# halide/Halide

Measured on AMD Instinct MI355X. Metric: megapixels/sec local_laplacian 8-level fp32 4K, higher is better.
Workload: dtype f32; 1 GPU; apps/local_laplacian J=8 levels=8 alpha=1/7 beta=1, u16 RGB planar 3840x2160; distinct_frames_per_gpu=8, lut_cached=True, streams_per_gpu=4, frame_scheduling=4 frame-queue streams, boundary=C ABI local_laplacian(halide_buffer_t*,int32,float,float,halide_buffer_t*), rccl_ranks=1, parallelism=frames sharded over 1 GPU(s), no data-path collective

## Files before the change

### halide_amd/csrc/local_laplacian.hip

```cpp
#include "hlmi_device_math.h"
#include "hlmi_internal.h"

#include <atomic>
#include <mutex>
#include <optional>
#include <stdlib.h>
#include <string.h>
#include <type_traits>

using namespace hlmi;

namespace {

constexpr int J = 8;
constexpr int MAX_K = 32;
constexpr int STRIP = 126;
constexpr int KCH = 8;
constexpr int D0_THREADS = 256;

struct Level {
    int lox, loy;
    int w, h;
    int ws;
    size_t ps;
    int rx0, rx1, ry0, ry1;
    bool odd;
    int nsx;
};

#ifndef HLMI_LL_PROBE
#define HLMI_LL_PROBE 0
#endif
#if HLMI_LL_PROBE
__device__ unsigned long long g_probe[32];
#define LL_PROBE_T(var) const unsigned long long var = wall_clock64()
#define LL_PROBE_ADD(slot, val) do { if ((threadIdx.x & 63) == 0) atomicAdd(&g_probe[slot], (unsigned long long)(val)); } while (0)
#else
#define LL_PROBE_T(var)
#define LL_PROBE_ADD(slot, val)
#endif

#ifndef HLMI_LL_RESIDENCY
#define HLMI_LL_RESIDENCY 0
#endif
#if HLMI_LL_RESIDENCY
__device__ int g_res[2][4096];
__device__ unsigned long long g_res_hist[16];
struct ResidencyProbe {
    int kind, slot;
    bool on;
    __device__ explicit ResidencyProbe(int k) : kind(k), slot(0), on(threadIdx.x == 0) {
        if (on) {
            unsigned hw, xcc;
            asm volatile("s_getreg_b32 %0, hwreg(HW_REG_HW_ID)" : "=s"(hw));
            asm volatile("s_getreg_b32 %0, hwreg(HW_REG_XCC_ID)" : "=s"(xcc));
            slot = (int)(((xcc & 0xfu) << 8) | ((hw >> 8) & 0xffu));
            const int own = atomicAdd(&g_res[kind][slot], 1);
            const int other = atomicAdd(&g_res[1 - kind][slot], 0);
            atomicAdd(&g_res_hist[8 * kind + min(other, 3)], 1ull);
            atomicAdd(&g_res_hist[8 * kind + 4 + min(own, 3)], 1ull);
        }
    }
    __device__ ~ResidencyProbe() {
        if (on) atomicSub(&g_res[kind][slot], 1);
    }
};
#define LL_RESIDENCY(kind) ResidencyProbe residency_probe_(kind)
#else
#define LL_RESIDENCY(kind)
#endif

struct Geometry {
    int K, half;
    float Km1, inv_Km1;
    int ix0, ix1, iy0, iy1;
};

__global__ void ll_remap_lut(float *lut, int half, float alpha) {
    int i = blockIdx.x * blockDim.x + threadIdx.x;
    if (i > 2 * half) return;
    float fx = (float)(i - half) * (1.0f / 256.0f);
    lut[i] = (alpha * fx) * dev::halide_exp(((-fx) * fx) * 0.5f);
}

__device__ __forceinline__ int xcd_block() {
    const int nb8 = gridDim.x >> 3, b = blockIdx.x;
    return (b < (nb8 << 3)) ? (b & 7) * nb8 + (b >> 3) : b;
}

__device__ __forceinline__ float down4(float a, float b, float c, float d) {
    return (dev::mad(3.0f, b + c, a) + d) * 0.125f;
}
__device__ __forceinline__ float down4_raw(float a, float b, float c, float d) { return dev::mad(3.0f, b + c, a) + d; }
__device__ __forceinline__ float down4_tail(float a, float b, float c, float d) {
    return (dev::mad(3.0f, b + c, a) + d) * 0.015625f;
}

__device__ __forceinline__ float gray_from(uint16_t r, uint16_t g, uint16_t b) {
    constexpr float s = (float)(1.0 / 65535.0);
    constexpr float C0 = (float)((double)s * (double)0.299f), C1 = (float)((double)s * (double)0.587f),
                    C2 = (float)((double)s * (double)0.114f);
    return dev::mad((float)b, C2, dev::mad2((float)r, C0, (float)g, C1));
}
__device__ __forceinline__ int idx_of(float gray, float Km1, int half) {
    return dev::clampi((int)((gray * Km1) * 256.0f), 0, half);
}
template<bool B1 = false>
__device__ __forceinline__ float g0_val(float gray, float level, float beta, float l) {
    return B1 ? ((gray - level) + level) + l : dev::mad(beta, gray - level, level) + l;
}

__device__ __forceinline__ float lane_prev(float v) {
    return __builtin_bit_cast(float, __builtin_amdgcn_update_dpp(0, __builtin_bit_cast(int, v), 0x138, 0xf, 0xf, true));
}
__device__ __forceinline__ float lane_next(float v) {
    return __builtin_bit_cast(float, __builtin_amdgcn_update_dpp(0, __builtin_bit_cast(int, v), 0x130, 0xf, 0xf, true));
}
__global__ void ll_dpp_probe(int *ok) {
    float v = (float)threadIdx.x;
    float p = lane_prev(v), n = lane_next(v);
    bool good = (threadIdx.x == 0 || p == v - 1.0f) && (threadIdx.x == 63 || n == v + 1.0f);
    unsigned long long m = __ballot(good);
    if (threadIdx.x == 0) *ok = (m == ~0ull) ? 1 : 0;
}

template<bool ODD>
__device__ __forceinline__ float2 hpair(const float (&dy)[4]) {
    if (!ODD) {
        float left = lane_prev(dy[3]);
        float right = lane_next(dy[0]);
        float o0 = down4_tail(left, dy[0], dy[1], dy[2]);
        float o1 = down4_tail(dy[1], dy[2], dy[3], right);
        float o2 = lane_next(o0);
        return make_float2(o1, o2);
    } else {
        float r0 = lane_next(dy[0]), r1 = lane_next(dy[1]);
        float o0 = down4_tail(dy[0], dy[1], dy[2], dy[3]);
        float o1 = down4_tail(dy[2], dy[3], r0, r1);
        return make_float2(o0, o1);
    }
}

struct QuadSel {
    int oq;
    int sel[4];
    bool plain;
};
__device__ __forceinline__ QuadSel quad_sel(int o, int w) {
    QuadSel q;
    q.oq = dev::clampi(o, 0, (w - 1) & ~3);
#pragma unroll
    for (int i = 0; i < 4; i++) q.sel[i] = dev::clampi(o + i, 0, w - 1) - q.oq;
    q.plain = (o >= 0) && (o + 3 <= w - 1);
    return q;
}
template<typename T>
__device__ __forceinline__ T pick4(T x, T y, T z, T w, int s) {
    T lo = (s & 1) ? y : x, hi = (s & 1) ? w : z;
    return (s & 2) ? hi : lo;
}

typedef unsigned short us4_t __attribute__((ext_vector_type(4)));
template<bool NT = false>
__device__ __forceinline__ ushort4 ld_frame4(const uint16_t *p) {
    if (NT) {
        us4_t v = __builtin_nontemporal_load(reinterpret_cast<const us4_t *>(p));
        return make_ushort4(v.x, v.y, v.z, v.w);
    }
    return *reinterpret_cast<const ushort4 *>(p);
}
template<bool NT = false>
__device__ __forceinline__ ushort2 ld_frame2(const void *sbase, uint32_t byte_off) {
    const uint32_t *q = reinterpret_cast<const uint32_t *>(reinterpret_cast<const char *>(sbase) + byte_off);
    const uint32_t w = NT ? __builtin_nontemporal_load(q) : *q;
    return make_ushort2((uint16_t)(w & 0xffffu), (uint16_t)(w >> 16));
}
template<bool NT = false>
__device__ __forceinline__ void st_frame2(void *p, uint16_t a, uint16_t b) {
    const uint32_t w = (uint32_t)a | ((uint32_t)b << 16);
    if (NT) __builtin_nontemporal_store(w, reinterpret_cast<uint32_t *>(p));
    else *reinterpret_cast<uint32_t *>(p) = w;
}

struct Raw {
    ushort4 c0, c1, c2;
};
struct Levels {
    float v[MAX_K];
};

template<bool VEC, bool NT = false>
__device__ __forceinline__ void load_raw(Raw &r, const uint16_t *__restrict__ rp, long co0, long co1, long co2,
                                         int oq, const int (&xo)[4]) {
    if (VEC) {
        r.c0 = ld_frame4<NT>(rp + co0 + oq);
        r.c1 = ld_frame4<NT>(rp + co1 + oq);
        r.c2 = ld_frame4<NT>(rp + co2 + oq);
    } else {
        r.c0 = make_ushort4(rp[co0 + xo[0]], rp[co0 + xo[1]], rp[co0 + xo[2]], rp[co0 + xo[3]]);
        r.c1 = make_ushort4(rp[co1 + xo[0]], rp[co1 + xo[1]], rp[co1 + xo[2]], rp[co1 + xo[3]]);
        r.c2 = make_ushort4(rp[co2 + xo[0]], rp[co2 + xo[1]], rp[co2 + xo[2]], rp[co2 + xo[3]]);
    }
}

template<bool ODD, bool VEC, bool LUT_LDS, bool B1>
__global__ __launch_bounds__(D0_THREADS, 2) void ll_down0(const uint16_t *__restrict__ in, long in_sy, long co0, long co1,
                                                   long co2, Geometry gm, Levels lev, float beta,
                                                   const float *__restrict__ lut_g, float *__restrict__ g1, int Xs,
                                                   int loy1, int w1, int h1, int ws1, size_t ps1, int nsx, int nsy,
                                                   int nunits) {
    extern __shared__ float slut[];
    if (LUT_LDS) {
        for (int i = threadIdx.x; i <= 2 * gm.half; i += D0_THREADS) slut[i] = lut_g[i];
        __syncthreads();
    }
    const float *lut = LUT_LDS ? slut : lut_g;
    const int wave = __builtin_amdgcn_readfirstlane(threadIdx.x >> 6);
    const int unit = xcd_block() * (D0_THREADS / 64) + wave;
    if (unit >= nunits) return;
    const int lane = threadIdx.x & 63;
    const int sy = unit % nsy, sx = unit / nsy;
    const int off = STRIP * sx + 2 * lane;
    const int P = Xs + off;
    const int q0 = ODD ? 2 * P - 1 : 2 * P - 2;
    const int iw = gm.ix1 - gm.ix0 + 1, ih = gm.iy1 - gm.iy0;
    const QuadSel qs = quad_sel(q0 - gm.ix0, iw);
    int xo[4];
#pragma unroll
    for (int i = 0; i < 4; i++) xo[i] = qs.oq + qs.sel[i];
    const bool edge_wave = VEC && __any(!qs.plain);
    const bool store_ok = (lane < 63) && (off < w1);
    const int t0 = (int)((long)sy * h1 / nsy), t1 = (int)((long)(sy + 1) * h1 / nsy) - 1;

    auto row_ptr = [&](int y_abs) -> const uint16_t * {
        return in + (long)(dev::clampi(y_abs - gm.iy0, 0, ih)) * in_sy;
    };

    for (int kb = 0; kb < gm.K; kb += KCH) {
        const int nk = min(KCH, gm.K - kb);
        const bool with_in = (kb == 0);
        const int lbase = gm.half - 256 * (kb + KCH - 1);
        float level[KCH];
#pragma unroll
        for (int kk = 0; kk < KCH; kk++) {
            const float lk = (float)(kb + kk) * gm.inv_Km1;
            level[kk] = kb + kk < MAX_K ? lev.v[kb + kk]
                                        : __builtin_bit_cast(float, __builtin_amdgcn_readfirstlane(__builtin_bit_cast(int, lk)));
            asm volatile("" : "+s"(level[kk]));
        }

        float a[KCH + 1][4], b[KCH + 1][4], a2[KCH + 1][4], b2[KCH + 1][4];
        auto gray_row = [&](const Raw &r, float (&gr)[4], int (&li)[4]) {
            const uint16_t rr[4] = {r.c0.x, r.c0.y, r.c0.z, r.c0.w};
            const uint16_t gg[4] = {r.c1.x, r.c1.y, r.c1.z, r.c1.w};
            const uint16_t bb[4] = {r.c2.x, r.c2.y, r.c2.z, r.c2.w};
            float g[4];
#pragma unroll
            for (int i = 0; i < 4; i++) g[i] = gray_from(rr[i], gg[i], bb[i]);
            if (edge_wave) {
#pragma unroll
                for (int i = 0; i < 4; i++) gr[i] = pick4(g[0], g[1], g[2], g[3], qs.sel[i]);
            } else {
#pragma unroll
                for (int i = 0; i < 4; i++) gr[i] = g[i];
            }
#pragma unroll
            for (int i = 0; i < 4; i++) li[i] = idx_of(gr[i], gm.Km1, gm.half) + lbase;
        };
        auto lut_issue = [&](int kk, const int (&l0)[4], const int (&l1)[4], float (&dst)[8]) {
#pragma unroll
            for (int i = 0; i < 4; i++) {
                dst[i] = lut[l0[i] + 256 * (KCH - 1 - kk)];
                dst[4 + i] = lut[l1[i] + 256 * (KCH - 1 - kk)];
            }
        };
        auto for_planes = [&](const float (&g0r)[4], const int (&l0)[4], const float (&g1r)[4], const int (&l1)[4],
                              auto &&F, auto &&G) {
            float lv[2][8];
            lut_issue(0, l0, l1, lv[0]);
#pragma unroll
            for (int kk = 0; kk <= KCH; kk++) {
                if (kk + 1 < KCH && kk + 1 < nk) lut_issue(kk + 1, l0, l1, lv[(kk + 1) & 1]);
                __builtin_amdgcn_sched_barrier(0);
                if (kk < KCH ? (kk < nk) : with_in) {
#pragma unroll
                    for (int i = 0; i < 4; i++) {
                        float v0 = kk < KCH ? g0_val<B1>(g0r[i], level[kk < KCH ? kk : 0], beta, lv[kk & 1][i]) : g0r[i];
                        float v1 = kk < KCH ? g0_val<B1>(g1r[i], level[kk < KCH ? kk : 0], beta, lv[kk & 1][4 + i]) : g1r[i];
                        F(kk, i, v0, v1);
                    }
                    G(kk);
                }
                __builtin_amdgcn_sched_barrier(0);
            }
        };

        const int T0 = loy1 + t0;
        {
            Raw ra, rb;
            load_raw<VEC>(ra, row_ptr(2 * T0 - 1), co0, co1, co2, qs.oq, xo);
            load_raw<VEC>(rb, row_ptr(2 * T0), co0, co1, co2, qs.oq, xo);
            float gra[4], grb[4];
            int la[4], lb[4];
            gray_row(ra, gra, la);
            gray_row(rb, grb, lb);
            for_planes(gra, la, grb, lb, [&](int kk, int i, float v0, float v1) { a[kk][i] = v0, b[kk][i] = v1; },
                       [&](int) {});
        }
        struct RowPair {
            float g0[4], g1[4];
        };
        Raw rc, rd;
        auto lut_pos = [&](const float (&g)[4], int (&l)[4]) {
#pragma unroll
            for (int i = 0; i < 4; i++) l[i] = idx_of(g[i], gm.Km1, gm.half) + lbase;
        };
        float2 *stage = reinterpret_cast<float2 *>(slut + (LUT_LDS ? ((2 * gm.half + 1 + 1) & ~1) : 0)) + threadIdx.x;
        auto step = [&](int t, const RowPair &cur, RowPair &nxt, float (&ia)[KCH + 1][4], float (&ib)[KCH + 1][4],
                        float (&oa)[KCH + 1][4], float (&ob)[KCH + 1][4]) {
            const int T = loy1 + t;
            int l0[4], l1[4];
            lut_pos(cur.g0, l0);
            lut_pos(cur.g1, l1);
            float dy[4];
            for_planes(cur.g0, l0, cur.g1, l1,
                       [&](int kk, int i, float cv, float dv) {
                           dy[i] = down4_raw(ia[kk][i], ib[kk][i], cv, dv);
                           oa[kk][i] = cv;
                           ob[kk][i] = dv;
                       },
                       [&](int kk) { stage[kk * D0_THREADS] = hpair<ODD>(dy); });
            if (t < t1) {
                int unused[4];
                gray_row(rc, nxt.g0, unused);
                gray_row(rd, nxt.g1, unused);
            }
            __builtin_amdgcn_sched_barrier(0);
            float *drow = g1 + (size_t)t * ws1 + off;
#pragma unroll
            for (int kk = 0; kk <= KCH; kk++) {
                if (kk < KCH ? (kk < nk) : with_in) {
                    const int plane = (kk < KCH) ? kb + kk : gm.K;
                    const float2 o = stage[kk * D0_THREADS];
                    if (store_ok) {
                        *reinterpret_cast<float2 *>(drow + (size_t)plane * ps1) = o;
                    }
                }
            }
            __builtin_amdgcn_sched_barrier(0);
            if (t + 1 < t1) {
                load_raw<VEC>(rc, row_ptr(2 * T + 5), co0, co1, co2, qs.oq, xo);
                load_raw<VEC>(rd, row_ptr(2 * T + 6), co0, co1, co2, qs.oq, xo);
            }
            __builtin_amdgcn_sched_barrier(0);
        };
        RowPair p0, p1;
        load_raw<VEC>(rc, row_ptr(2 * T0 + 1), co0, co1, co2, qs.oq, xo);
        load_raw<VEC>(rd, row_ptr(2 * T0 + 2), co0, co1, co2, qs.oq, xo);
        {
            int unused[4];
            gray_row(rc, p0.g0, unused);
            gray_row(rd, p0.g1, unused);
        }
        if (t0 < t1) {
            load_raw<VEC>(rc, row_ptr(2 * T0 + 3), co0, co1, co2, qs.oq, xo);
            load_raw<VEC>(rd, row_ptr(2 * T0 + 4), co0, co1, co2, qs.oq, xo);
        }
        for (int t = t0; t <= t1;) {
            step(t, p0, p1, a, b, a2, b2);
            if (++t > t1) break;
            step(t, p1, p0, a2, b2, a, b);
            ++t;
        }
    }
}

struct D01Args {
    const uint16_t *in;
    long in_sy, co0, co1, co2;
    float beta;
    const float *lut_g;
    float *g1;
    int so1, loy1, w1, h1, ws1;
    size_t ps1;
    float *g2;
    int so2, loy2, w2, h2, ws2;
    size_t ps2;
    int Pbase, S2, nsx, nsy, nunits;
    unsigned nsy_magic;
    int rows_base, rows_rem;
};
constexpr int D01_STATE = 2 * (KCH + 1) * 64;

template<bool ODD0, bool ODD1, bool B1, bool EXCH>
__global__ __launch_bounds__(D0_THREADS, 2) void ll_down01f(D01Args p, Geometry gm, Levels lev) {
    extern __shared__ float slut[];
    LL_PROBE_T(pt0);
    for (int i = threadIdx.x; i <= 2 * gm.half; i += D0_THREADS) slut[i] = p.lut_g[i];
    __syncthreads();
    LL_PROBE_T(pt1);
    const int wave = __builtin_amdgcn_readfirstlane(threadIdx.x >> 6);
    const int lane = threadIdx.x & 63;
    int sx, A, B;
    bool self_halo = true;
    bool publish = false;
    if (EXCH) {
        const int wg = xcd_block();
        sx = p.nsy_magic ? (int)__umulhi((unsigned)wg, p.nsy_magic) : wg;
        const int gy = wg - sx * p.nsy;
        const int GA = p.loy2 + gy * p.rows_base + min(gy, p.rows_rem);
        const int GB = GA + p.rows_base + (gy < p.rows_rem ? 1 : 0) - 1;
        const int n = (GB - GA + 1 + 1 + 3) >> 2;
        A = GA + wave * n, B = min(A + n - 1, GB);
        if (A > GB) {
            __syncthreads();
            return;
        }
        self_halo = !(wave < 3 && A + n <= GB);
        publish = wave > 0;
    } else {
        const int unit = xcd_block() * (D0_THREADS / 64) + wave;
        if (unit >= p.nunits) return;
        sx = p.nsy_magic ? (int)__umulhi((unsigned)unit, p.nsy_magic) : unit;
        const int sy = unit - sx * p.nsy;
        A = p.loy2 + sy * p.rows_base + min(sy, p.rows_rem);
        B = A + p.rows_base + (sy < p.rows_rem ? 1 : 0) - 1;
    }
    const int P = p.Pbase + 2 * p.S2 * sx + 2 * lane;
    const int q0 = ODD0 ? 2 * P - 1 : 2 * P - 2;
    const int iw = gm.ix1 - gm.ix0 + 1, ih = gm.iy1 - gm.iy0;
    const QuadSel qs = quad_sel(q0 - gm.ix0, iw);
    int xo[4];
#pragma unroll
    for (int i = 0; i < 4; i++) xo[i] = qs.oq + qs.sel[i];
    const bool edge_wave = __any(!qs.plain);
    const int T0 = 2 * A - 1, T1 = self_halo ? 2 * B + 2 : 2 * B;
    const int Ts0 = max(EXCH ? 2 * A - 1 : 2 * A, p.loy1), Ts1 = min(EXCH ? 2 * B : 2 * B + 1, p.loy1 + p.h1 - 1);
    const int off1 = P - p.so1;
    const bool st1_ok = lane < p.S2 && off1 >= 0 && off1 < p.w1;
    const int X2 = ODD1 ? (P + 1) >> 1 : P >> 1;
    const int off2 = X2 - p.so2;
    const bool st2_ok = (ODD1 ? lane < p.S2 : (lane >= 1 && lane <= p.S2)) && off2 >= 0 && off2 < p.w2;
    float2 *st2 = reinterpret_cast<float2 *>(slut + ((2 * gm.half + 2) & ~1)) + wave * D01_STATE + lane;
    float2 *pub_all = reinterpret_cast<float2 *>(slut + ((2 * gm.half + 2) & ~1)) + (D0_THREADS / 64) * D01_STATE + lane;
    float2 *pub_mine = pub_all + (wave - 1) * D01_STATE, *pub_next = pub_all + wave * D01_STATE;
    const int lbase = gm.half - 256 * (KCH - 1);
    float level[KCH];
#pragma unroll
    for (int kk = 0; kk < KCH; kk++) {
        level[kk] = lev.v[kk];
        asm volatile("" : "+v"(level[kk]));
    }
    auto walk = [&](auto edge_tag) {
    constexpr bool EDGE = decltype(edge_tag)::value;
#if HLMI_LL_PROBE
    unsigned long long pr_a0 = 0, pr_a = 0, pr_3 = 0;
#endif
    auto load_row = [&](Raw &r, int y_abs) {
        const uint16_t *rp = p.in + (long)(dev::clampi(y_abs - gm.iy0, 0, ih)) * p.in_sy;
        load_raw<true>(r, rp, p.co0, p.co1, p.co2, qs.oq, xo);
    };
    auto u16s = [&](const ushort4 &c, uint16_t (&o)[4]) {
        const uint2 w = __builtin_bit_cast(uint2, c);
        o[0] = (uint16_t)(w.x & 0xffffu), o[1] = (uint16_t)(w.x >> 16);
        o[2] = (uint16_t)(w.y & 0xffffu), o[3] = (uint16_t)(w.y >> 16);
    };
    struct Row {
        float g[4];
        int l[4];
    };
    auto prep_row = [&](const Raw &r, Row &o) {
        uint16_t rr[4], gg[4], bb[4];
        u16s(r.c0, rr), u16s(r.c1, gg), u16s(r.c2, bb);
#pragma unroll
        for (int i = 0; i < 4; i++) o.g[i] = gray_from(rr[i], gg[i], bb[i]);
        if (EDGE) {
            const float g0 = o.g[0], g1v = o.g[1], g2v = o.g[2], g3 = o.g[3];
#pragma unroll
            for (int i = 0; i < 4; i++) o.g[i] = pick4(g0, g1v, g2v, g3, qs.sel[i]);
        }
#pragma unroll
        for (int i = 0; i < 4; i++) {
            o.l[i] = (min((int)((o.g[i] * gm.Km1) * 256.0f), gm.half) + lbase) * 4;
            asm volatile("" : "+v"(o.l[i]));
        }
    };
    auto lut_issue = [&](int kk, const Row &r0, const Row &r1, float (&dst)[8]) {
#pragma unroll
        for (int i = 0; i < 4; i++) {
            dst[i] = *reinterpret_cast<const float *>(reinterpret_cast<const char *>(slut) + r0.l[i] + 1024 * (KCH - 1 - kk));
            dst[4 + i] = *reinterpret_cast<const float *>(reinterpret_cast<const char *>(slut) + r1.l[i] + 1024 * (KCH - 1 - kk));
        }
    };
    auto plane_vals = [&](int kk, const Row &r0, const Row &r1, const float (&lv)[8], float (&v0)[4], float (&v1)[4]) {
        if (kk < KCH) {
            const float L = level[kk < KCH ? kk : 0];
            float t[8];
#pragma unroll
            for (int i = 0; i < 4; i++) t[i] = r0.g[i] - L, t[4 + i] = r1.g[i] - L;
            if (!B1 && !dev::CANON_FMA) {
#pragma unroll
                for (int i = 0; i < 8; i++) t[i] = p.beta * t[i];
            }
#pragma unroll
            for (int i = 0; i < 8; i++) t[i] = (!B1 && dev::CANON_FMA) ? __builtin_fmaf(p.beta, t[i], L) : t[i] + L;
#pragma unroll
            for (int i = 0; i < 4; i++) v0[i] = t[i] + lv[i], v1[i] = t[4 + i] + lv[4 + i];
        } else {
#pragma unroll
            for (int i = 0; i < 4; i++) v0[i] = r0.g[i], v1[i] = r1.g[i];
        }
    };
    auto vpass = [&](const float (&ia)[4], const float (&ib)[4], const float (&c)[4], const float (&d)[4], float (&o)[4]) {
        float t[4];
#pragma unroll
        for (int i = 0; i < 4; i++) t[i] = ib[i] + c[i];
        if (!dev::CANON_FMA) {
#pragma unroll
            for (int i = 0; i < 4; i++) t[i] = 3.0f * t[i];
        }
#pragma unroll
        for (int i = 0; i < 4; i++) t[i] = dev::CANON_FMA ? __builtin_fmaf(3.0f, t[i], ia[i]) : ia[i] + t[i];
#pragma unroll
        for (int i = 0; i < 4; i++) o[i] = t[i] + d[i];
    };

    float a[KCH + 1][4], b[KCH + 1][4], a2[KCH + 1][4], b2[KCH + 1][4];
    Raw rc, rd;
    {
        Raw ra, rb;
        load_row(ra, 2 * T0 - 1);
        load_row(rb, 2 * T0);
        load_row(rc, 2 * T0 + 1);
        load_row(rd, 2 * T0 + 2);
#if HLMI_LL_PROBE
        LL_PROBE_T(ptA0);
        asm volatile("s_waitcnt vmcnt(0)" ::: "memory");
        LL_PROBE_T(ptA);
        pr_a0 = ptA0, pr_a = ptA;
#endif
        Row r0, r1;
        prep_row(ra, r0);
        prep_row(rb, r1);
        float lv[2][8];
        lut_issue(0, r0, r1, lv[0]);
#pragma unroll
        for (int kk = 0; kk <= KCH; kk++) {
            if (kk + 1 < KCH) lut_issue(kk + 1, r0, r1, lv[(kk + 1) & 1]);
            __builtin_amdgcn_sched_barrier(0);
            plane_vals(kk, r0, r1, lv[kk & 1], a[kk], b[kk]);
            __builtin_amdgcn_sched_barrier(0);
        }
    }
    auto step = [&](auto ph_tag, int T, const Row &c0, const Row &c1, Row &n0, Row &n1, float (&ia)[KCH + 1][4],
                    float (&ib)[KCH + 1][4], float (&oa)[KCH + 1][4], float (&ob)[KCH + 1][4], float2 *pub) {
        constexpr int PH = decltype(ph_tag)::value;
        float lv[2][8], dy[2][4];
        float2 res[KCH + 1];
        float2 sa, sb;
        const bool out2 = PH == 1 && T >= 2 * A + 2;
        float *d2 = p.g2 + (size_t)(((T - 2) >> 1) - p.loy2) * p.ws2 + off2;
        auto level2 = [&](int k) {
            const float2 c = res[k];
            if (PH == 0) {
                float2 pc;
                pc.x = dev::mad(3.0f, sb.x + c.x, sa.x);
                pc.y = dev::mad(3.0f, sb.y + c.y, sa.y);
                st2[(2 * k + 1) * 64] = pc;
                st2[(2 * k) * 64] = c;
            } else {
                const float rx = sb.x + c.x, ry = sb.y + c.y;
                float o;
                if (ODD1) {
                    const float nx = lane_next(rx), ny = lane_next(ry);
                    o = down4_tail(rx, ry, nx, ny);
                } else {
                    const float py = lane_prev(ry), nx = lane_next(rx);
                    o = down4_tail(py, rx, ry, nx);
                }
                if (out2 && st2_ok) d2[(size_t)k * p.ps2] = o;
                st2[(2 * k + 1) * 64] = c;
            }
        };
        auto state_issue = [&](int k) {
            if (PH == 0) sa = st2[(2 * k) * 64];
            sb = st2[(2 * k + 1) * 64];
        };
        lut_issue(0, c0, c1, lv[0]);
#pragma unroll
        for (int kk = 0; kk <= KCH; kk++) {
            if (kk > 0) state_issue(kk - 1);
            __builtin_amdgcn_sched_barrier(0);
            if (kk + 1 < KCH) lut_issue(kk + 1, c0, c1, lv[(kk + 1) & 1]);
            __builtin_amdgcn_sched_barrier(0);
            plane_vals(kk, c0, c1, lv[kk & 1], oa[kk], ob[kk]);
            vpass(ia[kk], ib[kk], oa[kk], ob[kk], dy[kk & 1]);
            if (kk > 0) {
                res[kk - 1] = hpair<ODD0>(dy[(kk - 1) & 1]);
                level2(kk - 1);
            }
            __builtin_amdgcn_sched_barrier(0);
        }
        state_issue(KCH);
        res[KCH] = hpair<ODD0>(dy[KCH & 1]);
        level2(KCH);
        prep_row(rc, n0);
        prep_row(rd, n1);
        __builtin_amdgcn_sched_barrier(0);
        if (T >= Ts0 && T <= Ts1) {
            float *drow = p.g1 + (size_t)(T - p.loy1) * p.ws1 + off1;
            if (st1_ok) {
#pragma unroll
                for (int kk = 0; kk <= KCH; kk++) *reinterpret_cast<float2 *>(drow + (size_t)kk * p.ps1) = res[kk];
            }
        }
        if (EXCH && pub) {
#pragma unroll
            for (int kk = 0; kk <= KCH; kk++) pub[kk * 64] = res[kk];
        }
        __builtin_amdgcn_sched_barrier(0);
        if (T + 1 < T1) {
            load_row(rc, 2 * T + 5);
            load_row(rd, 2 * T + 6);
        }
        __builtin_amdgcn_sched_barrier(0);
    };
    Row p0, p1, p2, p3;
    prep_row(rc, p0);
    prep_row(rd, p1);
    load_row(rc, 2 * T0 + 3);
    load_row(rd, 2 * T0 + 4);
    LL_PROBE_T(pt2);
    for (int T = T0; T <= T1; T += 2) {
        const bool first = EXCH && T == T0;
        step(std::integral_constant<int, 0>{}, T, p0, p1, p2, p3, a, b, a2, b2, first && publish ? pub_mine : nullptr);
        step(std::integral_constant<int, 1>{}, T + 1, p2, p3, p0, p1, a2, b2, a, b,
             first && publish ? pub_mine + (KCH + 1) * 64 : nullptr);
        if (first) __syncthreads();
#if HLMI_LL_PROBE
        if (first) { LL_PROBE_T(pt3); pr_3 = pt3; }
#endif
    }
    LL_PROBE_T(pt4);
    LL_PROBE_ADD(0, pt1 - pt0); LL_PROBE_ADD(1, 1); LL_PROBE_ADD(2, pt2 - pt1); LL_PROBE_ADD(3, pr_3 - pt2);
    LL_PROBE_ADD(16, pr_a - pr_a0); LL_PROBE_ADD(17, pr_a0 - pt1);
    LL_PROBE_ADD(4, pt4 - pt2); LL_PROBE_ADD(5, (T1 - T0 + 1)); LL_PROBE_ADD(6, pt4 - pt0);
    if (EXCH && !self_halo) {
        float *d2 = p.g2 + (size_t)(B - p.loy2) * p.ws2 + off2;
#pragma unroll
        for (int k = 0; k <= KCH; k++) {
            const float2 sa = st2[(2 * k) * 64], sb = st2[(2 * k + 1) * 64];
            const float2 c = pub_next[k * 64], d = pub_next[(KCH + 1 + k) * 64];
            const float rx = dev::mad(3.0f, sb.x + c.x, sa.x) + d.x, ry = dev::mad(3.0f, sb.y + c.y, sa.y) + d.y;
            float o;
            if (ODD1) {
                const float nx = lane_next(rx), ny = lane_next(ry);
                o = down4_tail(rx, ry, nx, ny);
            } else {
                const float py = lane_prev(ry), nx = lane_next(rx);
                o = down4_tail(py, rx, ry, nx);
            }
            if (st2_ok) d2[(size_t)k * p.ps2] = o;
        }
    }
    };
    if (edge_wave) walk(std::true_type{});
    else walk(std::false_type{});
}

struct D01EArgs {
    D01Args d;
    float *outl0;
    int oy0, oh;
    unsigned nsx_magic;
};
typedef float f2 __attribute__((ext_vector_type(2)));
__device__ __forceinline__ f2 f2s(float v) { return f2{v, v}; }
__device__ __forceinline__ f2 fma2(f2 a, f2 b, f2 c) { return __builtin_elementwise_fma(a, b, c); }
__device__ __forceinline__ f2 mad_2(f2 a, f2 b, f2 c) { return dev::CANON_FMA ? fma2(a, b, c) : a * b + c; }
__device__ __forceinline__ f2 mad2_2(f2 a, f2 b, f2 c, f2 d) { return dev::CANON_FMA ? fma2(a, b, c * d) : a * b + c * d; }

template<bool ODD0, bool ODD1, bool B1, bool EXCH, bool NT>
__global__ __launch_bounds__(D0_THREADS, 2) void ll_down01e(D01EArgs pe, Geometry gm, Levels lev) {
    const D01Args &p = pe.d;
    LL_RESIDENCY(0);
    extern __shared__ float slut[];
    for (int i = threadIdx.x; i <= 2 * gm.half; i += D0_THREADS) slut[i] = p.lut_g[i];
    __syncthreads();
    const int wave = __builtin_amdgcn_readfirstlane(threadIdx.x >> 6);
    const int lane = threadIdx.x & 63;
    int sx, A, B;
    bool self_halo = true;
    bool publish = false;
    if (EXCH) {
        const int wg = xcd_block();
        const int gy = pe.nsx_magic ? (int)__umulhi((unsigned)wg, pe.nsx_magic) : wg;
        sx = wg - gy * p.nsx;
        const int GA = p.loy2 + gy * p.rows_base + min(gy, p.rows_rem);
        const int GB = GA + p.rows_base + (gy < p.rows_rem ? 1 : 0) - 1;
        const int n = (GB - GA + 1 + 1 + 3) >> 2;
        A = GA + wave * n, B = min(A + n - 1, GB);
        if (A > GB) {
            __syncthreads();
            return;
        }
        self_halo = !(wave < 3 && A + n <= GB);
        publish = wave > 0;
    } else {
        const int unit = xcd_block() * (D0_THREADS / 64) + wave;
        if (unit >= p.nunits) return;
        sx = p.nsy_magic ? (int)__umulhi((unsigned)unit, p.nsy_magic) : unit;
        const int sy = unit - sx * p.nsy;
        A = p.loy2 + sy * p.rows_base + min(sy, p.rows_rem);
        B = A + p.rows_base + (sy < p.rows_rem ? 1 : 0) - 1;
    }
    const int P = p.Pbase + 2 * p.S2 * sx + 2 * lane;
    const int q0 = ODD0 ? 2 * P - 1 : 2 * P - 2;
    const int iw = gm.ix1 - gm.ix0 + 1, ih = gm.iy1 - gm.iy0;
    const QuadSel qs = quad_sel(q0 - gm.ix0, iw);
    int xo[4];
#pragma unroll
    for (int i = 0; i < 4; i++) xo[i] = qs.oq + qs.sel[i];
    const bool edge_wave = __any(!qs.plain);
    const int T0 = 2 * A - 1, T1 = self_halo ? 2 * B + 2 : 2 * B;
    const int Ts0 = max(EXCH ? 2 * A - 1 : 2 * A, p.loy1), Ts1 = min(EXCH ? 2 * B : 2 * B + 1, p.loy1 + p.h1 - 1);
    const int off1 = P - p.so1;
    const bool st1_ok = lane < p.S2 && off1 >= 0 && off1 < p.w1;
    const int X2 = ODD1 ? (P + 1) >> 1 : P >> 1;
    const int off2 = X2 - p.so2;
    const bool st2_ok = (ODD1 ? lane < p.S2 : (lane >= 1 && lane <= p.S2)) && off2 >= 0 && off2 < p.w2;
    const bool em_ok = lane >= 1 && lane <= p.S2 && q0 >= gm.ix0 && q0 + 3 <= gm.ix1;
    float *const em_col = pe.outl0 + (q0 - gm.ix0);
    f2 *st2 = reinterpret_cast<f2 *>(slut + ((2 * gm.half + 2) & ~1)) + wave * D01_STATE + lane;
    f2 *pub_all = reinterpret_cast<f2 *>(slut + ((2 * gm.half + 2) & ~1)) + (D0_THREADS / 64) * D01_STATE + lane;
    f2 *pub_mine = pub_all + (wave - 1) * D01_STATE, *pub_next = pub_all + wave * D01_STATE;
    const int lbase = gm.half - 256 * (KCH - 1);
    float level[KCH];
#pragma unroll
    for (int kk = 0; kk < KCH; kk++) {
        level[kk] = lev.v[kk];
        asm volatile("" : "+v"(level[kk]));
    }
    auto walk = [&](auto edge_tag) {
    constexpr bool EDGE = decltype(edge_tag)::value;
    auto load_row = [&](Raw &r, int y_abs) {
        const uint16_t *rp = p.in + (long)(dev::clampi(y_abs - gm.iy0, 0, ih)) * p.in_sy;
        load_raw<true, NT>(r, rp, p.co0, p.co1, p.co2, qs.oq, xo);
    };
    auto u16s = [&](const ushort4 &c, uint16_t (&o)[4]) {
        const uint2 w = __builtin_bit_cast(uint2, c);
        o[0] = (uint16_t)(w.x & 0xffffu), o[1] = (uint16_t)(w.x >> 16);
        o[2] = (uint16_t)(w.y & 0xffffu), o[3] = (uint16_t)(w.y >> 16);
    };
    struct Row {
        f2 g[2];
        int l[4];
    };
    auto prep_row = [&](const Raw &r, Row &o) {
        uint16_t rr[4], gg[4], bb[4];
        u16s(r.c0, rr), u16s(r.c1, gg), u16s(r.c2, bb);
        constexpr float s = (float)(1.0 / 65535.0);
        constexpr float C0 = (float)((double)s * (double)0.299f), C1 = (float)((double)s * (double)0.587f),
                        C2 = (float)((double)s * (double)0.114f);
#pragma unroll
        for (int h = 0; h < 2; h++) {
            const f2 fr = {(float)rr[h], (float)rr[h + 2]}, fg = {(float)gg[h], (float)gg[h + 2]}, fb = {(float)bb[h], (float)bb[h + 2]};
            o.g[h] = mad_2(fb, f2s(C2), mad2_2(fr, f2s(C0), fg, f2s(C1)));
        }
        if (EDGE) {
            const float g0 = o.g[0].x, g1v = o.g[1].x, g2v = o.g[0].y, g3 = o.g[1].y;
            o.g[0].x = pick4(g0, g1v, g2v, g3, qs.sel[0]), o.g[1].x = pick4(g0, g1v, g2v, g3, qs.sel[1]);
            o.g[0].y = pick4(g0, g1v, g2v, g3, qs.sel[2]), o.g[1].y = pick4(g0, g1v, g2v, g3, qs.sel[3]);
        }
#pragma unroll
        for (int h = 0; h < 2; h++) {
            const f2 t = (o.g[h] * gm.Km1) * 256.0f;
            o.l[h] = (min((int)t.x, gm.half) + lbase) * 4;
            o.l[h + 2] = (min((int)t.y, gm.half) + lbase) * 4;
        }
#pragma unroll
        for (int i = 0; i < 4; i++) asm volatile("" : "+v"(o.l[i]));
    };
    auto lut_issue = [&](int kk, const Row &r0, const Row &r1, f2 (&dst)[4]) {
        auto rd = [&](int l) {
            return *reinterpret_cast<const float *>(reinterpret_cast<const char *>(slut) + l + 1024 * (KCH - 1 - kk));
        };
        dst[0].x = rd(r0.l[0]), dst[1].x = rd(r0.l[1]), dst[0].y = rd(r0.l[2]), dst[1].y = rd(r0.l[3]);
        dst[2].x = rd(r1.l[0]), dst[3].x = rd(r1.l[1]), dst[2].y = rd(r1.l[2]), dst[3].y = rd(r1.l[3]);
    };
    auto plane_vals = [&](int kk, const Row &r0, const Row &r1, const f2 (&lv)[4], f2 (&v0)[2], f2 (&v1)[2]) {
        if (B1 && kk == 0) {
            v0[0] = r0.g[0] + lv[0], v0[1] = r0.g[1] + lv[1], v1[0] = r1.g[0] + lv[2], v1[1] = r1.g[1] + lv[3];
        } else if (kk < KCH) {
            const f2 L = f2s(level[kk < KCH ? kk : 0]);
            f2 t[4] = {r0.g[0] - L, r0.g[1] - L, r1.g[0] - L, r1.g[1] - L};
            if (!B1 && !dev::CANON_FMA) {
#pragma unroll
                for (int i = 0; i < 4; i++) t[i] = p.beta * t[i];
            }
#pragma unroll
            for (int i = 0; i < 4; i++) t[i] = (!B1 && dev::CANON_FMA) ? fma2(f2s(p.beta), t[i], L) : t[i] + L;
            v0[0] = t[0] + lv[0], v0[1] = t[1] + lv[1], v1[0] = t[2] + lv[2], v1[1] = t[3] + lv[3];
        } else {
            v0[0] = r0.g[0], v0[1] = r0.g[1], v1[0] = r1.g[0], v1[1] = r1.g[1];
        }
    };
    auto vpass = [&](const f2 (&ia)[2], const f2 (&ib)[2], const f2 (&c)[2], const f2 (&d)[2], f2 (&o)[2]) {
        f2 t[2] = {ib[0] + c[0], ib[1] + c[1]};
        if (dev::CANON_FMA) {
            t[0] = fma2(f2s(3.0f), t[0], ia[0]), t[1] = fma2(f2s(3.0f), t[1], ia[1]);
        } else {
            t[0] = 3.0f * t[0], t[1] = 3.0f * t[1];
            t[0] = ia[0] + t[0], t[1] = ia[1] + t[1];
        }
        o[0] = t[0] + d[0], o[1] = t[1] + d[1];
    };
    auto hpair2 = [&](const f2 (&dy)[2]) {
        const float d4[4] = {dy[0].x, dy[1].x, dy[0].y, dy[1].y};
        const float2 r = hpair<ODD0>(d4);
        return f2{r.x, r.y};
    };
    struct EmPix {
        f2 lut, qa, qb, ta, tb;
        float lif;
    };
    auto em_gather = [&](const Row &n, int i, const f2 *rq, const f2 *rt, EmPix &g) {
        constexpr int COL[4] = {ODD0 ? -1 : -2, -1, ODD0 ? 0 : -1, 0};
        const uint32_t aq0 = (uint32_t)(size_t)rq, at0 = (uint32_t)(size_t)rt, alut = (uint32_t)(size_t)slut + 1024u * (KCH - 2);
        auto rd2 = [](uint32_t addr, auto swap_tag) {
            f2 v;
            if (decltype(swap_tag)::value) asm volatile("ds_read2st64_b32 %0, %1 offset0:4" : "=v"(v) : "v"(addr) : "memory");
            else asm volatile("ds_read2st64_b32 %0, %1 offset1:4" : "=v"(v) : "v"(addr) : "memory");
            return v;
        };
        constexpr std::false_type asc{};
        constexpr std::true_type desc{};
        const int pos = n.l[i] - lbase * 4;
        const int li = min(pos >> 10, KCH - 2);
        const uint32_t po = (uint32_t)(li << 10) + (uint32_t)(COL[i] * 4);
        g.lut = rd2(alut + (uint32_t)n.l[i] - (uint32_t)(li << 10), desc);
        if ((COL[i] & 1) == 0) {
            auto rd64 = [](uint32_t addr, auto plane1) {
                f2 v;
                if (decltype(plane1)::value) asm volatile("ds_read_b64 %0, %1 offset:1024" : "=v"(v) : "v"(addr) : "memory");
                else asm volatile("ds_read_b64 %0, %1" : "=v"(v) : "v"(addr) : "memory");
                return v;
            };
            g.qa = rd64(aq0 + po, asc), g.qb = rd64(aq0 + po, desc);
            g.ta = rd64(at0 + po, asc), g.tb = rd64(at0 + po, desc);
        } else {
            g.qa = rd2(aq0 + po, asc), g.qb = rd2(aq0 + po + 4u, asc);
            g.ta = rd2(at0 + po, asc), g.tb = rd2(at0 + po + 4u, asc);
        }
        g.lif = (float)li;
    };
    auto em_wait = [&](EmPix &g, auto after_tag) {
        constexpr int AFTER = decltype(after_tag)::value;
        static_assert(AFTER >= 0 && AFTER <= 3, "");
        if (AFTER == 0) asm volatile("s_waitcnt lgkmcnt(0)" : "+v"(g.lut), "+v"(g.qa), "+v"(g.qb), "+v"(g.ta), "+v"(g.tb));
        if (AFTER == 1) asm volatile("s_waitcnt lgkmcnt(5)" : "+v"(g.lut), "+v"(g.qa), "+v"(g.qb), "+v"(g.ta), "+v"(g.tb));
        if (AFTER == 2) asm volatile("s_waitcnt lgkmcnt(10)" : "+v"(g.lut), "+v"(g.qa), "+v"(g.qb), "+v"(g.ta), "+v"(g.tb));
        if (AFTER == 3) asm volatile("s_waitcnt lgkmcnt(15)" : "+v"(g.lut), "+v"(g.qa), "+v"(g.qb), "+v"(g.ta), "+v"(g.tb));
    };
    auto em_arith = [&](const Row &n, int i, const EmPix &g, auto yodd_tag) {
        constexpr bool YODD = decltype(yodd_tag)::value;
        const bool xodd = ODD0 ? (i & 1) == 0 : (i & 1) == 1;
        auto hl = [&](f2 fa, f2 fb) {
            if (xodd) return fma2(fb, f2s(0.25f), fa * 0.75f);
            return dev::CANON_FMA ? fma2(fb, f2s(0.75f), fa * 0.25f) : fma2(fa, f2s(0.25f), fb * 0.75f);
        };
        auto vl = [](f2 uq, f2 ut) {
            return (dev::CANON_FMA && !YODD) ? fma2(ut, f2s(0.75f), uq * 0.25f) : fma2(uq, f2s(0.25f), ut * 0.75f);
        };
        const float gr = n.g[i & 1][i >> 1];
        const float lf = gr * gm.Km1 - g.lif;
        const f2 lev = f2{g.lif, g.lif + 1.0f} * gm.inv_Km1;
        constexpr int COLP[4] = {ODD0 ? -1 : -2, -1, ODD0 ? 0 : -1, 0};
        f2 u;
        if ((COLP[i] & 1) == 0) {
            auto hls = [&](float fa, float fb) {
                if (xodd) return __builtin_fmaf(fb, 0.25f, fa * 0.75f);
                return dev::CANON_FMA ? __builtin_fmaf(fb, 0.75f, fa * 0.25f) : __builtin_fmaf(fa, 0.25f, fb * 0.75f);
            };
            auto vls = [](float uq, float ut) {
                return (dev::CANON_FMA && !YODD) ? __builtin_fmaf(ut, 0.75f, uq * 0.25f) : __builtin_fmaf(uq, 0.25f, ut * 0.75f);
            };
            u = f2{vls(hls(g.qa.x, g.qa.y), hls(g.ta.x, g.ta.y)), vls(hls(g.qb.x, g.qb.y), hls(g.tb.x, g.tb.y))};
        } else {
            u = vl(hl(g.qa, g.qb), hl(g.ta, g.tb));
        }
        const f2 g2 = f2s(gr);
        const f2 l = (B1 ? ((g2 - lev) + lev) + g.lut : mad_2(f2s(p.beta), g2 - lev, lev) + g.lut) - u;
        if (dev::CANON_FMA) return __builtin_fmaf(1.0f - lf, l.x, lf * l.y);
        const f2 m = f2{1.0f - lf, lf} * l;
        return m.x + m.y;
    };
    constexpr std::true_type row_odd{};
    constexpr std::false_type row_even{};
    constexpr std::integral_constant<int, 0> after0{};
    constexpr std::integral_constant<int, 1> after1{};
    constexpr std::integral_constant<int, 2> after2{};
    constexpr std::integral_constant<int, 3> after3{};
    auto emit_row = [&](const Row &n, const f2 *rq, const f2 *rt, float (&r)[4], auto yodd_tag) {
        EmPix g[4];
#pragma unroll
        for (int i = 0; i < 4; i++) em_gather(n, i, rq, rt, g[i]);
        em_wait(g[0], after3), r[0] = em_arith(n, 0, g[0], yodd_tag);
        em_wait(g[1], after2), r[1] = em_arith(n, 1, g[1], yodd_tag);
        em_wait(g[2], after1), r[2] = em_arith(n, 2, g[2], yodd_tag);
        em_wait(g[3], after0), r[3] = em_arith(n, 3, g[3], yodd_tag);
    };
    auto emit_store = [&](int y, const float (&r)[4]) {
        if (em_ok && y >= pe.oy0 && y < pe.oy0 + pe.oh) {
            typedef float f4_t __attribute__((ext_vector_type(4)));
            f4_t *const dst = reinterpret_cast<f4_t *>(em_col + (size_t)(y - pe.oy0) * iw);
            if (NT) __builtin_nontemporal_store(f4_t{r[0], r[1], r[2], r[3]}, dst);
            else *dst = f4_t{r[0], r[1], r[2], r[3]};
        }
    };
#if HLMI_LL_PROBE
    unsigned long long pr_planes = 0, pr_emit = 0, pr_prep = 0, pr_steps = 0;
    LL_PROBE_T(pe0);
    const unsigned long long pc0 = __builtin_readcyclecounter();
#endif
    f2 a[KCH + 1][2], b[KCH + 1][2], a2[KCH + 1][2], b2[KCH + 1][2];
    f2 pcr[KCH + 1];
    Raw rc, rd;
    {
        Raw ra, rb;
        load_row(ra, 2 * T0 - 1);
        load_row(rb, 2 * T0);
        load_row(rc, 2 * T0 + 1);
        load_row(rd, 2 * T0 + 2);
        Row r0, r1;
        prep_row(ra, r0);
        prep_row(rb, r1);
        f2 lv[2][4];
        lut_issue(0, r0, r1, lv[0]);
#pragma unroll
        for (int kk = 0; kk <= KCH; kk++) {
            if (kk + 1 < KCH) lut_issue(kk + 1, r0, r1, lv[(kk + 1) & 1]);
            __builtin_amdgcn_sched_barrier(0);
            plane_vals(kk, r0, r1, lv[kk & 1], a[kk], b[kk]);
            __builtin_amdgcn_sched_barrier(0);
        }
    }
    auto step = [&](auto ph_tag, int T, const Row &c0, const Row &c1, Row &n0, Row &n1, f2 (&ia)[KCH + 1][2],
                    f2 (&ib)[KCH + 1][2], f2 (&oa)[KCH + 1][2], f2 (&ob)[KCH + 1][2], f2 *pub) {
        constexpr int PH = decltype(ph_tag)::value;
        f2 lv[2][4], dy[2][2];
        f2 res[KCH + 1];
        f2 sa, sb;
        const bool out2 = PH == 1 && T >= 2 * A + 2;
        float *d2 = p.g2 + (size_t)(((T - 2) >> 1) - p.loy2) * p.ws2 + off2;
        LL_PROBE_T(ps0);
        auto level2 = [&](int k) {
            const f2 c = res[k];
            if (PH == 0) {
                pcr[k] = mad_2(f2s(3.0f), sb + c, sa);
                st2[(2 * k) * 64] = c;
            } else {
                const f2 r = pcr[k] + c;
                float o;
                if (ODD1) {
                    const float nx = lane_next(r.x), ny = lane_next(r.y);
                    o = down4_tail(r.x, r.y, nx, ny);
                } else {
                    const float py = lane_prev(r.y), nx = lane_next(r.x);
                    o = down4_tail(py, r.x, r.y, nx);
                }
                if (out2 && st2_ok) d2[(size_t)k * p.ps2] = o;
                st2[(2 * k + 1) * 64] = c;
            }
        };
        auto state_issue = [&](int k) {
            if (PH == 0) sa = st2[(2 * k) * 64], sb = st2[(2 * k + 1) * 64];
        };
        lut_issue(0, c0, c1, lv[0]);
#pragma unroll
        for (int kk = 0; kk <= KCH; kk++) {
            if (kk > 0) state_issue(kk - 1);
            __builtin_amdgcn_sched_barrier(0);
            if (kk + 1 < KCH) lut_issue(kk + 1, c0, c1, lv[(kk + 1) & 1]);
            __builtin_amdgcn_sched_barrier(0);
            plane_vals(kk, c0, c1, lv[kk & 1], oa[kk], ob[kk]);
            vpass(ia[kk], ib[kk], oa[kk], ob[kk], dy[kk & 1]);
            if (kk > 0) {
                res[kk - 1] = hpair2(dy[(kk - 1) & 1]);
                level2(kk - 1);
            }
            __builtin_amdgcn_sched_barrier(0);
        }
        asm volatile("" ::: "memory");
        __builtin_amdgcn_wave_barrier();
        __builtin_amdgcn_sched_barrier(0);
        f2 *const rowT = st2 + (PH == 0 ? 0 : 64), *const rowP = st2 + (PH == 0 ? 64 : 0);
        const bool st1_row = T >= Ts0 && T <= Ts1;
        const bool em_rows = T >= 2 * A && T <= 2 * B + 1;
        EmPix eg[4];
        if (em_rows) {
#pragma unroll
            for (int i = 0; i < 4; i++) em_gather(n0, i, rowT, rowP, eg[i]);
        }
        __builtin_amdgcn_sched_barrier(0);
        state_issue(KCH);
        res[KCH] = hpair2(dy[KCH & 1]);
        level2(KCH);
        if (EXCH && pub) {
#pragma unroll
            for (int kk = 0; kk <= KCH; kk++) pub[(2 * kk) * 64] = res[kk];
        }
        asm volatile("" ::: "memory");
        __builtin_amdgcn_sched_barrier(0);
        LL_PROBE_T(ps1);
        float2 s0 = make_float2(0.0f, 0.0f), s1 = s0;
        const f2 sK = res[KCH];
        if (st1_row) {
            const int lx = dev::clampi((int)(sK.x * gm.Km1), 0, KCH - 2), ly = dev::clampi((int)(sK.y * gm.Km1), 0, KCH - 2);
            const float *fx = reinterpret_cast<const float *>(rowT) + (lx << 8), *fy = reinterpret_cast<const float *>(rowT) + (ly << 8) + 1;
            s0 = make_float2(fx[0], fy[0]), s1 = make_float2(fx[256], fy[256]);
        }
        float eo[4] = {0.0f, 0.0f, 0.0f, 0.0f}, ee[4] = {0.0f, 0.0f, 0.0f, 0.0f};
        if (em_rows) {
            EmPix fg[4];
            em_wait(eg[0], after3), eo[0] = em_arith(n0, 0, eg[0], row_odd);
            __builtin_amdgcn_sched_barrier(0);
            em_gather(n1, 0, rowP, rowT, fg[0]);
            __builtin_amdgcn_sched_barrier(0);
            em_wait(eg[1], after3), eo[1] = em_arith(n0, 1, eg[1], row_odd);
            __builtin_amdgcn_sched_barrier(0);
            em_gather(n1, 1, rowP, rowT, fg[1]);
            __builtin_amdgcn_sched_barrier(0);
            em_wait(eg[2], after3), eo[2] = em_arith(n0, 2, eg[2], row_odd);
            __builtin_amdgcn_sched_barrier(0);
            em_gather(n1, 2, rowP, rowT, fg[2]);
            __builtin_amdgcn_sched_barrier(0);
            em_wait(eg[3], after3), eo[3] = em_arith(n0, 3, eg[3], row_odd);
            __builtin_amdgcn_sched_barrier(0);
            em_gather(n1, 3, rowP, rowT, fg[3]);
            __builtin_amdgcn_sched_barrier(0);
            em_wait(fg[0], after3), ee[0] = em_arith(n1, 0, fg[0], row_even);
            em_wait(fg[1], after2), ee[1] = em_arith(n1, 1, fg[1], row_even);
            em_wait(fg[2], after1), ee[2] = em_arith(n1, 2, fg[2], row_even);
            em_wait(fg[3], after0), ee[3] = em_arith(n1, 3, fg[3], row_even);
        }
        asm volatile("" ::: "memory");
        __builtin_amdgcn_sched_barrier(0);
        LL_PROBE_T(ps2);
        prep_row(rc, n0);
        prep_row(rd, n1);
        __builtin_amdgcn_sched_barrier(0);
        if (st1_row && st1_ok) {
            float *drow = p.g1 + (size_t)(T - p.loy1) * p.ws1 + off1;
            *reinterpret_cast<float2 *>(drow) = s0;
            *reinterpret_cast<float2 *>(drow + p.ps1) = s1;
            *reinterpret_cast<f2 *>(drow + (size_t)KCH * p.ps1) = sK;
        }
        if (em_rows) {
            emit_store(2 * T - 1, eo);
            emit_store(2 * T, ee);
        }
        __builtin_amdgcn_sched_barrier(0);
        if (T + 1 < T1) {
            load_row(rc, 2 * T + 5);
            load_row(rd, 2 * T + 6);
        }
        __builtin_amdgcn_sched_barrier(0);
#if HLMI_LL_PROBE
        LL_PROBE_T(ps3);
        pr_planes += ps1 - ps0, pr_emit += ps2 - ps1, pr_prep += ps3 - ps2, pr_steps += 1;
#endif
    };
    Row p0, p1, p2, p3;
    prep_row(rc, p0);
    prep_row(rd, p1);
    load_row(rc, 2 * T0 + 3);
    load_row(rd, 2 * T0 + 4);
    for (int T = T0; T <= T1; T += 2) {
        const bool first = EXCH && T == T0;
        step(std::integral_constant<int, 0>{}, T, p0, p1, p2, p3, a, b, a2, b2, first && publish ? pub_mine : nullptr);
        step(std::integral_constant<int, 1>{}, T + 1, p2, p3, p0, p1, a2, b2, a, b, first && publish ? pub_mine + 64 : nullptr);
        if (first) __syncthreads();
    }
#if HLMI_LL_PROBE
    LL_PROBE_T(pe1);
#endif
    if (EXCH && !self_halo) {
        float *d2 = p.g2 + (size_t)(B - p.loy2) * p.ws2 + off2;
#pragma unroll
        for (int k = 0; k <= KCH; k++) {
            const f2 sa = st2[(2 * k) * 64], sb = st2[(2 * k + 1) * 64];
            const f2 c = pub_next[(2 * k) * 64], d = pub_next[(2 * k + 1) * 64];
            const f2 r = mad_2(f2s(3.0f), sb + c, sa) + d;
            float o;
            if (ODD1) {
                const float nx = lane_next(r.x), ny = lane_next(r.y);
                o = down4_tail(r.x, r.y, nx, ny);
            } else {
                const float py = lane_prev(r.y), nx = lane_next(r.x);
                o = down4_tail(py, r.x, r.y, nx);
            }
            if (st2_ok) d2[(size_t)k * p.ps2] = o;
        }
        {
            float eo[4], ee[4];
            emit_row(p2, pub_next, st2 + 64, eo, row_odd);
            emit_row(p3, st2 + 64, pub_next, ee, row_even);
            emit_store(4 * B + 1, eo);
            emit_store(4 * B + 2, ee);
        }
    }
#if HLMI_LL_PROBE
    LL_PROBE_T(pe2);
    LL_PROBE_ADD(27, __builtin_readcyclecounter() - pc0);
    LL_PROBE_ADD(28, pe2 - pe0);
    LL_PROBE_ADD(20, pr_planes); LL_PROBE_ADD(21, pr_emit); LL_PROBE_ADD(22, pr_prep); LL_PROBE_ADD(23, pr_steps);
    LL_PROBE_ADD(24, 1); LL_PROBE_ADD(25, pe1 - pe0); LL_PROBE_ADD(26, pe2 - pe1);
#endif
    };
    if (edge_wave) walk(std::true_type{});
    else walk(std::false_type{});
}

struct StripArgs {
    const float *src;
    int slox, sloy, sw, sh, sws;
    size_t sps;
    float *dst;
    int Xs, dloy, dw, dh, dws;
    size_t dps;
    int nsx, nsy, nunits;
};
template<bool ODD>
__device__ __forceinline__ void down_strip_unit(const StripArgs &a, int unit, int lane) {
    const int sy = unit % a.nsy, rest = unit / a.nsy, sx = rest % a.nsx, plane = rest / a.nsx;
    const int off = STRIP * sx + 2 * lane;
    const int P = a.Xs + off;
    const QuadSel qs = quad_sel((ODD ? 2 * P - 1 : 2 * P - 2) - a.slox, a.sw);
    const bool edge_wave = __any(!qs.plain);
    const bool store_ok = (lane < 63) && (off < a.dw);
    const int t0 = (int)((long)sy * a.dh / a.nsy), t1 = (int)((long)(sy + 1) * a.dh / a.nsy) - 1;
    const float *sp = a.src + (size_t)plane * a.sps + qs.oq;
    float *dp = a.dst + (size_t)plane * a.dps + off;
    auto row = [&](int y_abs) -> float4 {
        float4 v = *reinterpret_cast<const float4 *>(sp + (size_t)dev::clampi(y_abs - a.sloy, 0, a.sh - 1) * a.sws);
        if (edge_wave) {
            v = make_float4(pick4(v.x, v.y, v.z, v.w, qs.sel[0]), pick4(v.x, v.y, v.z, v.w, qs.sel[1]),
                            pick4(v.x, v.y, v.z, v.w, qs.sel[2]), pick4(v.x, v.y, v.z, v.w, qs.sel[3]));
        }
        return v;
    };
    const int T0 = a.dloy + t0;
    float4 ra = row(2 * T0 - 1), rb = row(2 * T0), rc = row(2 * T0 + 1), rd = row(2 * T0 + 2);
    for (int t = t0; t <= t1; t++) {
        const int T = a.dloy + t;
        float4 nc = rc, nd = rd;
        if (t < t1) {
            nc = row(2 * T + 3);
            nd = row(2 * T + 4);
        }
        float dy[4] = {down4_raw(ra.x, rb.x, rc.x, rd.x), down4_raw(ra.y, rb.y, rc.y, rd.y), down4_raw(ra.z, rb.z, rc.z, rd.z),
                       down4_raw(ra.w, rb.w, rc.w, rd.w)};
        float2 o = hpair<ODD>(dy);
        if (store_ok) *reinterpret_cast<float2 *>(dp + (size_t)t * a.dws) = o;
        ra = rc, rb = rd, rc = nc, rd = nd;
    }
}
template<bool ODD>
__global__ __launch_bounds__(256) void ll_down_strip(StripArgs a) {
    const int wave = __builtin_amdgcn_readfirstlane(threadIdx.x >> 6);
    const int unit = xcd_block() * 4 + wave;
    if (unit >= a.nunits) return;
    down_strip_unit<ODD>(a, unit, threadIdx.x & 63);
}

constexpr int S2_RPU = 2;
constexpr int S2_NT = 2 * S2_RPU + 2;
constexpr int S2_NSRC = 2 * S2_NT + 2;
struct Strip2Args {
    const float *src;
    int slox, sloy, sw, sh, sws;
    size_t sps;
    float *g1;
    int so1, loy1, w1, h1, ws1;
    size_t ps1;
    float *g2;
    int so2, loy2, w2, h2, ws2;
    size_t ps2;
    int Pbase, S2, nsx, nsy, nunits;
};
template<bool ODD0, bool ODD1>
__global__ __launch_bounds__(256) void ll_down_strip2(Strip2Args p) {
    const int wave = __builtin_amdgcn_readfirstlane(threadIdx.x >> 6);
    const int unit = xcd_block() * 4 + wave;
    if (unit >= p.nunits) return;
    const int lane = threadIdx.x & 63;
    const int sy = unit % p.nsy, rest = unit / p.nsy, sx = rest % p.nsx, plane = rest / p.nsx;
    const int A = p.loy2 + sy * S2_RPU, B = min(A + S2_RPU - 1, p.loy2 + p.h2 - 1);
    const int P = p.Pbase + 2 * p.S2 * sx + 2 * lane;
    const QuadSel qs = quad_sel((ODD0 ? 2 * P - 1 : 2 * P - 2) - p.slox, p.sw);
    const bool edge_wave = __any(!qs.plain);
    const int T0 = 2 * A - 1;
    const int Ts0 = max(2 * A, p.loy1), Ts1 = min(2 * B + 1, p.loy1 + p.h1 - 1);
    const int off1 = P - p.so1;
    const bool st1_ok = lane < p.S2 && off1 >= 0 && off1 < p.w1;
    const int X2 = ODD1 ? (P + 1) >> 1 : P >> 1;
    const int off2 = X2 - p.so2;
    const bool st2_ok = (ODD1 ? lane < p.S2 : (lane >= 1 && lane <= p.S2)) && off2 >= 0 && off2 < p.w2;
    const float *sp = p.src + (size_t)plane * p.sps + qs.oq;
    float4 r[S2_NSRC];
#pragma unroll
    for (int i = 0; i < S2_NSRC; i++) r[i] = *reinterpret_cast<const float4 *>(sp + (size_t)dev::clampi(2 * T0 - 1 + i - p.sloy, 0, p.sh - 1) * p.sws);
    if (edge_wave) {
#pragma unroll
        for (int i = 0; i < S2_NSRC; i++) {
            const float4 v = r[i];
            r[i] = make_float4(pick4(v.x, v.y, v.z, v.w, qs.sel[0]), pick4(v.x, v.y, v.z, v.w, qs.sel[1]),
                               pick4(v.x, v.y, v.z, v.w, qs.sel[2]), pick4(v.x, v.y, v.z, v.w, qs.sel[3]));
        }
    }
    float *d1 = p.g1 + (size_t)plane * p.ps1 + off1, *d2 = p.g2 + (size_t)plane * p.ps2 + off2;
    float2 s0 = make_float2(0.0f, 0.0f), s1 = s0, pc = s0;
#pragma unroll
    for (int t = 0; t < S2_NT; t++) {
        const int T = T0 + t;
        const float4 a = r[2 * t], b = r[2 * t + 1], c = r[2 * t + 2], d = r[2 * t + 3];
        const float dy[4] = {down4_raw(a.x, b.x, c.x, d.x), down4_raw(a.y, b.y, c.y, d.y), down4_raw(a.z, b.z, c.z, d.z),
                             down4_raw(a.w, b.w, c.w, d.w)};
        const float2 res = hpair<ODD0>(dy);
        if (T >= Ts0 && T <= Ts1 && st1_ok) *reinterpret_cast<float2 *>(d1 + (size_t)(T - p.loy1) * p.ws1) = res;
        if ((t & 1) == 0) {
            pc.x = dev::mad(3.0f, s1.x + res.x, s0.x);
            pc.y = dev::mad(3.0f, s1.y + res.y, s0.y);
            s0 = res;
        } else {
            const float rx = pc.x + res.x, ry = pc.y + res.y;
            float o;
            if (ODD1) {
                const float nx = lane_next(rx), ny = lane_next(ry);
                o = down4_tail(rx, ry, nx, ny);
            } else {
                const float py = lane_prev(ry), nx = lane_next(rx);
                o = down4_tail(py, rx, ry, nx);
            }
            const int Y = (T - 2) >> 1;
            if (T >= 2 * A + 2 && Y <= B && st2_ok) d2[(size_t)(Y - p.loy2) * p.ws2] = o;
            s1 = res;
        }
    }
}

struct UpTaps {
    float aa, ab, ba, bb;
};
__device__ __forceinline__ UpTaps up_taps(const float *__restrict__ f, int lox, int loy, int ws, int X, int Y) {
    const int xa = dev::fdiv2(X + 1) - lox, xb = dev::fdiv2(X - 1) - lox;
    const int ya = dev::fdiv2(Y + 1) - loy, yb = dev::fdiv2(Y - 1) - loy;
    UpTaps t;
    t.aa = f[(size_t)ya * ws + xa], t.ab = f[(size_t)ya * ws + xb];
    t.ba = f[(size_t)yb * ws + xa], t.bb = f[(size_t)yb * ws + xb];
    return t;
}
__device__ __forceinline__ float up_from(const UpTaps &t, int X, int Y) {
    const float wx = (float)(dev::fmod2(X) * 2 + 1) * 0.25f, wy = (float)(dev::fmod2(Y) * 2 + 1) * 0.25f;
    const float ua = dev::lerpf(t.aa, t.ab, wx);
    const float ub = dev::lerpf(t.ba, t.bb, wx);
    return dev::lerpf(ua, ub, wy);
}
__device__ __forceinline__ float up_at(const float *__restrict__ f, int lox, int loy, int ws, int X, int Y) {
    return up_from(up_taps(f, lox, loy, ws, X, Y), X, Y);
}

__device__ __forceinline__ float top_value(const float *__restrict__ g, size_t ps, size_t o, int K, float Km1) {
    float level = g[(size_t)K * ps + o] * Km1;
    int li = dev::clampi((int)level, 0, K - 2);
    float lf = level - (float)li;
    return dev::mad2(1.0f - lf, g[(size_t)li * ps + o], lf, g[(size_t)(li + 1) * ps + o]);
}
template<bool SEL = false>
__device__ __forceinline__ float outl_value(const float *__restrict__ g, int ws, size_t ps, int lox, int loy,
                                            const float *__restrict__ gc, int cws, size_t cps, int clox, int cloy,
                                            int X, int Y, int K, float Km1) {
    size_t o = (size_t)(Y - loy) * ws + (X - lox);
    float level = g[(size_t)K * ps + o] * Km1;
    int li = dev::clampi((int)level, 0, K - 2);
    float lf = level - (float)li;
    float l0 = g[(SEL ? 0 : (size_t)li * ps) + o] - up_at(gc + (size_t)li * cps, clox, cloy, cws, X, Y);
    float l1 = g[(SEL ? ps : (size_t)(li + 1) * ps) + o] - up_at(gc + (size_t)(li + 1) * cps, clox, cloy, cws, X, Y);
    return dev::mad2(1.0f - lf, l0, lf, l1);
}

__global__ void ll_top(const float *__restrict__ g, int ws, size_t ps, int lox, int loy, int rx0, int ry0, int rw,
                       int rh, int K, float Km1, float *__restrict__ out) {
    int x = blockIdx.x * blockDim.x + threadIdx.x, y = blockIdx.y;
    if (x >= rw || y >= rh) return;
    size_t o = (size_t)(ry0 + y - loy) * ws + (rx0 + x - lox);
    out[o] = top_value(g, ps, o, K, Km1);
}

struct UpArgs {
    const float *g;
    int ws;
    size_t ps;
    int lox, loy;
    const float *gc, *outc;
    int cws;
    size_t cps;
    int clox, cloy, rx0, ry0, rw, rh, K;
    float Km1;
    float *out;
};
template<bool SEL>
__device__ __forceinline__ void up_pixel(const UpArgs &a, int x, int y) {
    if (x >= a.rw || y >= a.rh) return;
    int X = a.rx0 + x, Y = a.ry0 + y;
    size_t o = (size_t)(Y - a.loy) * a.ws + (X - a.lox);
    float outL = outl_value<SEL>(a.g, a.ws, a.ps, a.lox, a.loy, a.gc, a.cws, a.cps, a.clox, a.cloy, X, Y, a.K, a.Km1);
    a.out[o] = up_at(a.outc, a.clox, a.cloy, a.cws, X, Y) + outL;
}
template<bool SEL = false>
__global__ __launch_bounds__(256) void ll_up(UpArgs a) {
    up_pixel<SEL>(a, blockIdx.x * blockDim.x + threadIdx.x, blockIdx.y);
}

struct DevLevel {
    float *g, *out;
    int lox, loy, w, h, ws;
    unsigned ps;
    int rx0, ry0, rw, rh;
};
struct CoarseArgs {
    DevLevel lv[J];
    int K;
    float Km1;
};

constexpr int DM_T = 4;
__host__ __device__ constexpr int dm_win(int depth_below) {
    int w = DM_T;
    for (int i = 0; i < depth_below; i++) w = 2 * w + 2;
    return w;
}
struct Range2 { int x0, x1, y0, y1; };
__device__ __forceinline__ Range2 clamp_to_box(const DevLevel &L, int x0, int x1, int y0, int y1) {
    Range2 r;
    r.x0 = dev::clampi(x0, L.lox, L.lox + L.w - 1), r.x1 = dev::clampi(x1, L.lox, L.lox + L.w - 1);
    r.y0 = dev::clampi(y0, L.loy, L.loy + L.h - 1), r.y1 = dev::clampi(y1, L.loy, L.loy + L.h - 1);
    return r;
}
template<int DEPTH>
__device__ __forceinline__ void down_multi_tile(const CoarseArgs &a, int ntx, int nty, int b) {
    constexpr int W1 = dm_win(DEPTH - 1), W2 = DEPTH >= 2 ? dm_win(DEPTH - 2) : 1, W3 = DEPTH >= 3 ? dm_win(DEPTH - 3) : 1,
                  W4 = DEPTH >= 4 ? dm_win(DEPTH - 4) : 1;
    __shared__ float tile1[W1 * W1], tile2[W2 * W2], tile3[W3 * W3], tile4[W4 * W4];
    float *const tiles[5] = {nullptr, tile1, tile2, tile3, tile4};
    const int ws_[5] = {0, W1, W2, W3, W4};
    const int tx = b % ntx, ty = (b / ntx) % nty, plane = b / (ntx * nty);
    Range2 win[5], own[5];
    {
        const DevLevel &T = a.lv[DEPTH];
        win[DEPTH] = own[DEPTH] = clamp_to_box(T, T.lox + tx * DM_T, T.lox + tx * DM_T + DM_T - 1, T.loy + ty * DM_T,
                                               T.loy + ty * DM_T + DM_T - 1);
#pragma unroll
        for (int d = DEPTH - 1; d >= 1; d--) {
            const DevLevel &L = a.lv[d];
            win[d] = clamp_to_box(L, 2 * win[d + 1].x0 - 1, 2 * win[d + 1].x1 + 2, 2 * win[d + 1].y0 - 1, 2 * win[d + 1].y1 + 2);
            own[d] = clamp_to_box(L, 2 * own[d + 1].x0, 2 * own[d + 1].x1 + 1, 2 * own[d + 1].y0, 2 * own[d + 1].y1 + 1);
        }
    }
#pragma unroll
    for (int d = 1; d <= DEPTH; d++) {
        const DevLevel &L = a.lv[d], &Sx = a.lv[d - 1];
        const Range2 w = win[d], o = own[d];
        const int nx = w.x1 - w.x0 + 1, n = nx * (w.y1 - w.y0 + 1);
        float *const dst = tiles[d];
        const float *const src_g = Sx.g + (size_t)plane * Sx.ps;
        const float *const src_t = tiles[d - 1];
        const Range2 pw = win[d == 1 ? 1 : d - 1];
        const int pnx = ws_[d == 1 ? 1 : d - 1];
        for (int e0 = threadIdx.x; e0 < n; e0 += 512) {
            float r[2][4][4];
            int X[2], Y[2], yy[2];
            bool ok[2];
#pragma unroll
            for (int u = 0; u < 2; u++) {
                const int e = e0 + 256 * u, ec = min(e, n - 1);
                ok[u] = e < n;
                yy[u] = ec / nx, X[u] = w.x0 + (ec - yy[u] * nx), Y[u] = w.y0 + yy[u];
#pragma unroll
                for (int i = 0; i < 4; i++) {
#pragma unroll
                    for (int k = 0; k < 4; k++) {
                        const int qx = dev::clampi(2 * X[u] - 1 + i, Sx.lox, Sx.lox + Sx.w - 1);
                        const int qy = dev::clampi(2 * Y[u] - 1 + k, Sx.loy, Sx.loy + Sx.h - 1);
                        r[u][i][k] = (d == 1) ? src_g[(size_t)(qy - Sx.loy) * Sx.ws + (qx - Sx.lox)]
                                              : src_t[(qy - pw.y0) * pnx + (qx - pw.x0)];
                    }
                }
            }
#pragma unroll
            for (int u = 0; u < 2; u++) {
                float v[4];
#pragma unroll
                for (int i = 0; i < 4; i++) v[i] = down4_raw(r[u][i][0], r[u][i][1], r[u][i][2], r[u][i][3]);
                const float val = down4_tail(v[0], v[1], v[2], v[3]);
                if (ok[u]) {
                    dst[yy[u] * ws_[d] + (X[u] - w.x0)] = val;
                    if (X[u] >= o.x0 && X[u] <= o.x1 && Y[u] >= o.y0 && Y[u] <= o.y1) {
                        L.g[(size_t)plane * L.ps + (size_t)(Y[u] - L.loy) * L.ws + (X[u] - L.lox)] = val;
                    }
                }
            }
        }
        if (d < DEPTH) __syncthreads();
    }
}
template<int DEPTH>
__global__ __launch_bounds__(256) void ll_down_multi(CoarseArgs a, int ntx, int nty) {
    down_multi_tile<DEPTH>(a, ntx, nty, (int)blockIdx.x);
}

constexpr int UM_T = 16;
__host__ __device__ constexpr int um_win(int d) {
    int w = UM_T;
    for (int i = 0; i < d; i++) w = w / 2 + 2;
    return w;
}
__host__ __device__ constexpr int um_off(int d) {
    int o = 0;
    for (int i = 0; i < d; i++) o += um_win(i) * um_win(i);
    return o;
}
static_assert(UM_T * UM_T <= 256 && um_win(1) * um_win(1) <= 256, "ll_up_multi: a level's region of a tile exceeds the workgroup");
template<int TOP>
__device__ __forceinline__ void up_multi_tile(const CoarseArgs &a, int ntx, int b) {
    __shared__ float tl[um_off(TOP + 1)];
    const int tx = b % ntx, ty = b / ntx;
    Range2 reg[TOP + 1];
    {
        const DevLevel &L = a.lv[0];
        reg[0].x0 = L.rx0 + tx * UM_T, reg[0].x1 = min(reg[0].x0 + UM_T - 1, L.rx0 + L.rw - 1);
        reg[0].y0 = L.ry0 + ty * UM_T, reg[0].y1 = min(reg[0].y0 + UM_T - 1, L.ry0 + L.rh - 1);
#pragma unroll
        for (int d = 1; d <= TOP; d++) {
            reg[d].x0 = dev::fdiv2(reg[d - 1].x0 - 1), reg[d].x1 = dev::fdiv2(reg[d - 1].x1 + 1);
            reg[d].y0 = dev::fdiv2(reg[d - 1].y0 - 1), reg[d].y1 = dev::fdiv2(reg[d - 1].y1 + 1);
        }
    }
    int eX[TOP + 1], eY[TOP + 1];
    bool act[TOP + 1];
    size_t eo[TOP + 1];
    float lvl[TOP + 1];
#pragma unroll
    for (int d = 0; d <= TOP; d++) {
        const DevLevel &L = a.lv[d];
        const Range2 r = reg[d];
        const int nx = r.x1 - r.x0 + 1, n = nx * (r.y1 - r.y0 + 1);
        act[d] = (int)threadIdx.x < n;
        const int e = act[d] ? (int)threadIdx.x : 0, yy = e / nx;
        eX[d] = r.x0 + (e - yy * nx), eY[d] = r.y0 + yy;
        eo[d] = (size_t)(eY[d] - L.loy) * L.ws + (eX[d] - L.lox);
        lvl[d] = L.g[(size_t)a.K * L.ps + eo[d]];
    }
    __builtin_amdgcn_sched_barrier(0);
    float lf[TOP + 1], g0[TOP + 1], g1[TOP + 1];
    int lis[TOP + 1];
    UpTaps t0[TOP + 1], t1[TOP + 1];
    auto planes_of = [&](int d) {
        const float level = lvl[d] * a.Km1;
        lis[d] = dev::clampi((int)level, 0, a.K - 2);
        lf[d] = level - (float)lis[d];
    };
#pragma unroll
    for (int d = 0; d <= TOP; d++) {
        const DevLevel &L = a.lv[d];
        planes_of(d);
        const int li = lis[d];
        g0[d] = L.g[(size_t)li * L.ps + eo[d]], g1[d] = L.g[(size_t)(li + 1) * L.ps + eo[d]];
        if (d < TOP) {
            const DevLevel &C = a.lv[d + 1];
            t0[d] = up_taps(C.g + (size_t)li * C.ps, C.lox, C.loy, C.ws, eX[d], eY[d]);
            t1[d] = up_taps(C.g + (size_t)(li + 1) * C.ps, C.lox, C.loy, C.ws, eX[d], eY[d]);
        }
    }
    __builtin_amdgcn_sched_barrier(0);
#pragma unroll
    for (int d = 0; d <= TOP; d++) {
        float v;
        if (d == TOP) {
            v = dev::mad2(1.0f - lf[d], g0[d], lf[d], g1[d]);
        } else {
            const float l0 = g0[d] - up_from(t0[d], eX[d], eY[d]);
            const float l1 = g1[d] - up_from(t1[d], eX[d], eY[d]);
            v = dev::mad2(1.0f - lf[d], l0, lf[d], l1);
        }
        if (act[d]) (tl + um_off(d))[(eY[d] - reg[d].y0) * um_win(d) + (eX[d] - reg[d].x0)] = v;
    }
    __syncthreads();
#pragma unroll
    for (int d = TOP - 1; d >= 0; d--) {
        const Range2 r = reg[d], c = reg[d + 1];
        const float *const ct = tl + um_off(d + 1);
        float *const tile = tl + um_off(d);
        const int cw = um_win(d + 1), tw = um_win(d);
        const int nx = r.x1 - r.x0 + 1, n = nx * (r.y1 - r.y0 + 1);
        for (int e = threadIdx.x; e < n; e += 256) {
            const int yy = e / nx, X = r.x0 + (e - yy * nx), Y = r.y0 + yy;
            const int xa = dev::fdiv2(X + 1) - c.x0, xb = dev::fdiv2(X - 1) - c.x0;
            const int ya = dev::fdiv2(Y + 1) - c.y0, yb = dev::fdiv2(Y - 1) - c.y0;
            const float wx = (float)(dev::fmod2(X) * 2 + 1) * 0.25f, wy = (float)(dev::fmod2(Y) * 2 + 1) * 0.25f;
            const float ua = dev::lerpf(ct[ya * cw + xa], ct[ya * cw + xb], wx);
            const float ub = dev::lerpf(ct[yb * cw + xa], ct[yb * cw + xb], wx);
            const float v = dev::lerpf(ua, ub, wy) + tile[yy * tw + (X - r.x0)];
            if (d == 0) {
                const DevLevel &L = a.lv[0];
                L.out[(size_t)(Y - L.loy) * L.ws + (X - L.lox)] = v;
            } else {
                tile[yy * tw + (X - r.x0)] = v;
            }
        }
        if (d > 0) __syncthreads();
    }
}
template<int TOP>
__global__ __launch_bounds__(256) void ll_up_multi(CoarseArgs a, int ntx) {
    up_multi_tile<TOP>(a, ntx, (int)blockIdx.x);
}



struct Up0Args {
    const uint16_t *in;
    long in_sy;
    long gco[3];
    long cco[3];
    const float *lut_g, *g1, *out1;
    int lox1, loy1, ws1;
    size_t ps1;
    uint16_t *out;
    long out_sy, out_sc;
    int ox0, oy0, ow, oh, nc, RU;
    int same_ch;
    float beta;
    const float *g2, *out2;
    int lox2, loy2, ws2;
    size_t ps2;
    int rx1_1;
    int rx0_1, ry0_1, ry1_1;
};

template<bool VEC, bool LUT_LDS>
__global__ __launch_bounds__(256) void ll_up0(Up0Args p, Geometry gm) {
    extern __shared__ float slut[];
    if (LUT_LDS) {
        for (int i = threadIdx.x; i <= 2 * gm.half; i += 256) slut[i] = p.lut_g[i];
        __syncthreads();
    }
    const float *lut = LUT_LDS ? slut : p.lut_g;
    const int wave = threadIdx.x >> 6, lane = threadIdx.x & 63;
    const int x = blockIdx.x * 256 + (wave & 1) * 128 + 2 * lane;
    const int y0 = blockIdx.y * (2 * p.RU) + (wave >> 1) * p.RU;
    if (x >= p.ow || y0 >= p.oh) return;
    const int npx = min(2, p.ow - x);
    const int y1 = min(y0 + p.RU, p.oh);
    const int X = p.ox0 + x;
    const bool vec = VEC && npx == 2;
    for (int y = y0; y < y1; y++) {
        const int Y = p.oy0 + y;
        const uint16_t *ip = p.in + (long)(Y - gm.iy0) * p.in_sy + (X - gm.ix0);
        uint16_t *op = p.out + (long)y * p.out_sy + x;
        uint16_t gch[3][2], cch[3][2];
        if (vec) {
#pragma unroll
            for (int c = 0; c < 3; c++) {
                ushort2 v = *reinterpret_cast<const ushort2 *>(ip + p.gco[c]);
                gch[c][0] = v.x, gch[c][1] = v.y;
            }
        } else {
#pragma unroll
            for (int c = 0; c < 3; c++) {
                gch[c][0] = ip[p.gco[c]];
                gch[c][1] = npx == 2 ? ip[p.gco[c] + 1] : gch[c][0];
            }
        }
        if (p.same_ch) {
#pragma unroll
            for (int c = 0; c < 3; c++) cch[c][0] = gch[c][0], cch[c][1] = gch[c][1];
        } else {
#pragma unroll
            for (int c = 0; c < 3; c++) {
                if (c < p.nc) {
                    cch[c][0] = ip[p.cco[c]];
                    cch[c][1] = npx == 2 ? ip[p.cco[c] + 1] : cch[c][0];
                } else {
                    cch[c][0] = cch[c][1] = 0;
                }
            }
        }
        uint16_t res[3][2];
#pragma unroll
        for (int i = 0; i < 2; i++) {
            const int Xi = X + i;
            float gray = gray_from(gch[0][i], gch[1][i], gch[2][i]);
            float level = gray * gm.Km1;
            int li = dev::clampi((int)level, 0, gm.K - 2);
            float lf = level - (float)li;
            int idx = idx_of(gray, gm.Km1, gm.half);
            const float *lp = lut + (idx - 256 * li + gm.half);
            float lev0 = (float)li * gm.inv_Km1, lev1 = (float)(li + 1) * gm.inv_Km1;
            const float *gp = p.g1 + (size_t)li * p.ps1;
            float l0 = g0_val(gray, lev0, p.beta, lp[0]) - up_at(gp, p.lox1, p.loy1, p.ws1, Xi, Y);
            float l1 = g0_val(gray, lev1, p.beta, lp[-256]) - up_at(gp + p.ps1, p.lox1, p.loy1, p.ws1, Xi, Y);
            float outL = dev::mad2(1.0f - lf, l0, lf, l1);
            float og = (up_at(p.out1, p.lox1, p.loy1, p.ws1, Xi, Y) + outL) + 0.01f;
            float gr = gray + 0.01f;
#pragma unroll
            for (int c = 0; c < 3; c++) {
                float v = ((float)cch[c][i] * og) / gr;
                res[c][i] = (uint16_t)dev::clampf(v, 0.0f, 65535.0f);
            }
        }
        if (vec) {
#pragma unroll
            for (int c = 0; c < 3; c++) {
                if (c < p.nc) {
                    *reinterpret_cast<ushort2 *>(op + (long)c * p.out_sc) = make_ushort2(res[c][0], res[c][1]);
                }
            }
        } else {
#pragma unroll
            for (int c = 0; c < 3; c++) {
                if (c < p.nc) {
                    op[(long)c * p.out_sc] = res[c][0];
                    if (npx == 2) op[(long)c * p.out_sc + 1] = res[c][1];
                }
            }
        }
    }
}

struct __attribute__((packed, aligned(4))) F2U { float x, y; };
struct __attribute__((packed, aligned(4))) F3U { float x, y, z; };
template<typename T>
__device__ __forceinline__ T ld_su(const void *sbase, uint32_t byte_off) {
    return *reinterpret_cast<const T *>(reinterpret_cast<const char *>(sbase) + byte_off);
}

__device__ __forceinline__ void div3_by(const float (&n)[3], float d, float (&q)[3]) {
    float r = __builtin_amdgcn_rcpf(d);
    float e = __builtin_fmaf(-d, r, 1.0f);
    r = __builtin_fmaf(e, r, r);
#pragma unroll
    for (int i = 0; i < 3; i++) {
        float qq = n[i] * r;
        float t = __builtin_fmaf(-d, qq, n[i]);
        qq = __builtin_fmaf(t, r, qq);
        t = __builtin_fmaf(-d, qq, n[i]);
        q[i] = __builtin_fmaf(t, r, qq);
    }
}
__global__ void ll_div3_check(const float *n, const float *d, int count, int *bad) {
    int i = blockIdx.x * blockDim.x + threadIdx.x;
    if (i >= count) return;
    float nn[3] = {n[i], -n[i], n[i] * 3.0f}, q[3];
    div3_by(nn, d[i], q);
#pragma unroll
    for (int k = 0; k < 3; k++) {
        float ref = nn[k] / d[i];
        if (!(ref == q[k]) && !(ref != ref && q[k] != q[k])) atomicAdd(bad, 1);
    }
}

constexpr int U0_TW = 130, U0_TS = 131;
template<bool LUT_LDS, bool B1, bool FUSE1>
__global__ __launch_bounds__(256) void ll_up0f(Up0Args p, Geometry gm) {
    extern __shared__ float slut[];
    LL_PROBE_T(pt0);
    float *s_out1 = slut + (LUT_LDS ? ((2 * gm.half + 2) & ~1) : 0);
    if (LUT_LDS) {
        for (int i = threadIdx.x; i <= 2 * gm.half; i += 256) slut[i] = p.lut_g[i];
    }
    int cx0 = 0, cy0 = 0;
    if (FUSE1) {
        const int X0 = p.ox0 + (int)blockIdx.x * 256;
        const int Yw0 = p.oy0 + (int)blockIdx.y * (2 * p.RU);
        const int Yw1 = min(Yw0 + 2 * p.RU, p.oy0 + p.oh) - 1;
        cx0 = (X0 >> 1) - 1, cy0 = dev::fdiv2(Yw0 - 1);
        const int th = dev::fdiv2(Yw1 + 1) - cy0 + 1;
        for (int e = threadIdx.x; e < U0_TW * th; e += 256) {
            const int ty = e / U0_TW, tx = e - ty * U0_TW;
            const int cx = cx0 + tx, cy = cy0 + ty;
            if (cx > p.rx1_1) continue;
            const float outL = outl_value(p.g1, p.ws1, p.ps1, p.lox1, p.loy1, p.g2, p.ws2, p.ps2, p.lox2, p.loy2, cx, cy, gm.K, gm.Km1);
            s_out1[ty * U0_TS + tx] = up_at(p.out2, p.lox2, p.loy2, p.ws2, cx, cy) + outL;
        }
    }
    LL_PROBE_T(pt1);
    if (LUT_LDS || FUSE1) __syncthreads();
    LL_PROBE_T(pt2);
    const float *lut = LUT_LDS ? slut : p.lut_g;
    const int wave = __builtin_amdgcn_readfirstlane(threadIdx.x >> 6), lane = threadIdx.x & 63;
    const int x = blockIdx.x * 256 + (wave & 1) * 128 + 2 * lane;
    const int y0 = blockIdx.y * (2 * p.RU) + (wave >> 1) * p.RU;
    if (y0 >= p.oh || x >= p.ow) return;
    const int y1 = min(y0 + p.RU, p.oh);
    const int X = p.ox0 + x;
    const uint32_t colb = (uint32_t)((X >> 1) - 1 - p.lox1) * 4u;
    const uint32_t inb = (uint32_t)(X - gm.ix0) * 2u, outb = (uint32_t)x * 2u;
    const uint32_t psb = (uint32_t)p.ps1 * 4u;
    auto hl0 = [](float rm, float r0) {
        return dev::CANON_FMA ? __builtin_fmaf(r0, 0.75f, rm * 0.25f) : __builtin_fmaf(rm, 0.25f, r0 * 0.75f);
    };
    auto hl1 = [](float r0, float rp) { return __builtin_fmaf(rp, 0.25f, r0 * 0.75f); };
    struct Frame {
        ushort2 c0, c1, c2;
    };
    struct Prep {
        float chf[3][2];
        float gray[2], lf[2], lev0[2], lev1[2];
        float lut0[2], lut1[2];
        F3U OA, OB;
        float wq, wt;
    };
    struct Gath {
        F2U A0[2], B0[2], A1[2], Bp[2];
    };
    auto load_frame = [&](int y, Frame &f) {
        const uint16_t *irow = p.in + (long)(p.oy0 + min(y, y1 - 1) - gm.iy0) * p.in_sy;
        f.c0 = ld_frame2(irow + p.gco[0], inb), f.c1 = ld_frame2(irow + p.gco[1], inb), f.c2 = ld_frame2(irow + p.gco[2], inb);
    };
    auto vl = [](float uq, float ut, float wq, float wt) {
        return dev::CANON_FMA ? __builtin_fmaf(uq, wq, ut * wt) : __builtin_fmaf(uq, 0.25f, ut * 0.75f);
    };
    auto stage1 = [&](int yy, const Frame &f, Prep &s, Gath &g) {
        const int Y = p.oy0 + min(yy, y1 - 1);
        const int ya = dev::fdiv2(Y + 1) - p.loy1, yb = dev::fdiv2(Y - 1) - p.loy1;
        const bool yodd = dev::fmod2(Y) != 0;
        const int yq = (dev::CANON_FMA || yodd) ? ya : yb, yt = (dev::CANON_FMA || yodd) ? yb : ya;
        s.wq = yodd ? 0.25f : 0.75f, s.wt = yodd ? 0.75f : 0.25f;
        const float *ga = p.g1 + (size_t)yq * p.ws1, *gb = p.g1 + (size_t)yt * p.ws1;
        const uint16_t ch[3][2] = {{f.c0.x, f.c0.y}, {f.c1.x, f.c1.y}, {f.c2.x, f.c2.y}};
#pragma unroll
        for (int i = 0; i < 2; i++) {
            const float gray = gray_from(ch[0][i], ch[1][i], ch[2][i]);
            const float level = gray * gm.Km1;
            const int li = min((int)level, gm.K - 2);
            const float lif = (float)li;
            const int idx = min((int)(level * 256.0f), gm.half);
            const float *lp = lut + (idx - 256 * li + gm.half);
            const uint32_t pb = (uint32_t)li * psb + colb + 4u * i;
            g.A0[i] = ld_su<F2U>(ga, pb), g.B0[i] = ld_su<F2U>(gb, pb);
            g.A1[i] = ld_su<F2U>(ga, pb + psb), g.Bp[i] = ld_su<F2U>(gb, pb + psb);
            s.lut0[i] = lp[0], s.lut1[i] = lp[-256];
            s.gray[i] = gray, s.lf[i] = level - lif;
            s.lev0[i] = lif * gm.inv_Km1, s.lev1[i] = (lif + 1.0f) * gm.inv_Km1;
#pragma unroll
            for (int c = 0; c < 3; c++) s.chf[c][i] = (float)ch[c][i];
        }
        if (FUSE1) {
            const float *oa = s_out1 + (yq + p.loy1 - cy0) * U0_TS + (wave & 1) * 64 + lane;
            const float *ob = s_out1 + (yt + p.loy1 - cy0) * U0_TS + (wave & 1) * 64 + lane;
            s.OA.x = oa[0], s.OA.y = oa[1], s.OA.z = oa[2];
            s.OB.x = ob[0], s.OB.y = ob[1], s.OB.z = ob[2];
        } else {
            const float *oa = p.out1 + (size_t)yq * p.ws1, *ob = p.out1 + (size_t)yt * p.ws1;
            s.OA = ld_su<F3U>(oa, colb), s.OB = ld_su<F3U>(ob, colb);
        }
    };
    auto stage2 = [&](int y, const Prep &s, const Gath &g) {
        const float uo[2] = {vl(hl0(s.OA.x, s.OA.y), hl0(s.OB.x, s.OB.y), s.wq, s.wt), vl(hl1(s.OA.y, s.OA.z), hl1(s.OB.y, s.OB.z), s.wq, s.wt)};
        uint16_t res[3][2];
#pragma unroll
        for (int i = 0; i < 2; i++) {
            float u0, u1;
            if (i == 0) {
                u0 = vl(hl0(g.A0[i].x, g.A0[i].y), hl0(g.B0[i].x, g.B0[i].y), s.wq, s.wt), u1 = vl(hl0(g.A1[i].x, g.A1[i].y), hl0(g.Bp[i].x, g.Bp[i].y), s.wq, s.wt);
            } else {
                u0 = vl(hl1(g.A0[i].x, g.A0[i].y), hl1(g.B0[i].x, g.B0[i].y), s.wq, s.wt), u1 = vl(hl1(g.A1[i].x, g.A1[i].y), hl1(g.Bp[i].x, g.Bp[i].y), s.wq, s.wt);
            }
            const float l0 = g0_val<B1>(s.gray[i], s.lev0[i], p.beta, s.lut0[i]) - u0;
            const float l1 = g0_val<B1>(s.gray[i], s.lev1[i], p.beta, s.lut1[i]) - u1;
            const float outL = dev::mad2(1.0f - s.lf[i], l0, s.lf[i], l1);
            const float og = (uo[i] + outL) + 0.01f;
            const float gr = s.gray[i] + 0.01f;
            const float n[3] = {s.chf[0][i] * og, s.chf[1][i] * og, s.chf[2][i] * og};
            float q[3];
            div3_by(n, gr, q);
#pragma unroll
            for (int c = 0; c < 3; c++) res[c][i] = (uint16_t)__builtin_amdgcn_fmed3f(q[c], 0.0f, 65535.0f);
        }
        if (y < y1) {
            uint16_t *orow = p.out + (long)y * p.out_sy;
#pragma unroll
            for (int c = 0; c < 3; c++) st_frame2(reinterpret_cast<char *>(orow + (long)c * p.out_sc) + outb, res[c][0], res[c][1]);
        }
    };
    Frame f0, f1;
    Prep s0, s1;
    Gath g0, g1;
    load_frame(y0, f0);
    load_frame(y0 + 1, f1);
    stage1(y0, f0, s0, g0);
    for (int y = y0; y < y1; y += 2) {
        load_frame(y + 2, f0);
        __builtin_amdgcn_sched_barrier(0);
        stage1(y + 1, f1, s1, g1);
        __builtin_amdgcn_sched_barrier(0);
        stage2(y, s0, g0);
        __builtin_amdgcn_sched_barrier(0);
        load_frame(y + 3, f1);
        __builtin_amdgcn_sched_barrier(0);
        stage1(y + 2, f0, s0, g0);
        __builtin_amdgcn_sched_barrier(0);
        stage2(y + 1, s1, g1);
        __builtin_amdgcn_sched_barrier(0);
    }
    LL_PROBE_T(pt3);
    LL_PROBE_ADD(8, pt1 - pt0); LL_PROBE_ADD(9, pt2 - pt1); LL_PROBE_ADD(10, 1);
    LL_PROBE_ADD(11, pt3 - pt2); LL_PROBE_ADD(12, pt3 - pt0);
}

struct Up0HArgs {
    Up0Args u;
    const float *outl0;
    int l0_ws;
    int fuse2;
    const float *g3, *out3;
    int lox3, loy3, ws3;
    size_t ps3;
};
constexpr int U0H_PF = 4;
constexpr int U0H_T2 = 68;
template<bool NT, int CH = 2>
__global__ __launch_bounds__(256) void ll_up0h(Up0HArgs ph, Geometry gm) {
    const Up0Args &p = ph.u;
    LL_RESIDENCY(1);
    extern __shared__ float s_out1[];
    int bx, by;
    {
        const int b = (int)blockIdx.y * (int)gridDim.x + (int)blockIdx.x, nb8 = (int)(gridDim.x * gridDim.y) >> 3;
        const int lb = b < (nb8 << 3) ? (b & 7) * nb8 + (b >> 3) : b;
        by = lb / (int)gridDim.x, bx = lb - by * (int)gridDim.x;
    }
    const int X0 = p.ox0 + bx * 256;
    const int Yw0 = p.oy0 + by * (2 * p.RU);
    const int Yw1 = min(Yw0 + 2 * p.RU, p.oy0 + p.oh) - 1;
    const int cx0 = (X0 >> 1) - 1, cy0 = dev::fdiv2(Yw0 - 1);
    const int th = dev::fdiv2(Yw1 + 1) - cy0 + 1;
    float *const s_out2 = s_out1 + U0_TS * (p.RU + 2);
    const int cx1 = min(cx0 + U0_TW - 1, p.rx1_1);
    const int c2x0 = dev::fdiv2(cx0 - 1), c2y0 = dev::fdiv2(cy0 - 1);
    struct Taps32 {
        uint32_t b, a;
    };
    auto mul24 = [](uint32_t a, uint32_t b) { return (uint32_t)__umul24(a, b); };
    auto tap_bytes = [&](uint32_t row0, int y0, int lox, int ws, int X, int Y) {
        Taps32 t;
        t.b = (row0 + mul24((uint32_t)(dev::fdiv2(Y - 1) - y0), (uint32_t)ws) + (uint32_t)(dev::fdiv2(X - 1) - lox)) << 2;
        t.a = t.b + ((uint32_t)ws << 2);
        return t;
    };
    auto taps_at = [](const float *base, uint32_t plane_bytes, const Taps32 &t) {
        const F2U lo = ld_su<F2U>(base, plane_bytes + t.b), hi = ld_su<F2U>(base, plane_bytes + t.a);
        UpTaps r;
        r.bb = lo.x, r.ba = lo.y, r.ab = hi.x, r.aa = hi.y;
        return r;
    };
    const uint32_t ps1b = (uint32_t)p.ps1 * 4u, ps2b = (uint32_t)p.ps2 * 4u, ps3b = (uint32_t)ph.ps3 * 4u;
    if (ph.fuse2) {
        const int n2x = dev::fdiv2(cx1 + 1) - c2x0 + 1, n2y = dev::fdiv2(cy0 + th) - c2y0 + 1, n2 = n2x * n2y;
        const uint32_t m2 = (4194304u + (uint32_t)n2x - 1u) / (uint32_t)n2x;
        const int c3y0 = dev::fdiv2(c2y0 - 1);
        const uint32_t row2 = (uint32_t)((c2y0 - p.loy2) * p.ws2), row3 = (uint32_t)((c3y0 - ph.loy3) * ph.ws3);
        for (int e0 = threadIdx.x; e0 < n2; e0 += 256 * CH) {
            int X2[CH], Y2[CH];
            uint32_t ti[CH];
            bool ok[CH];
            uint32_t ob[CH];
            Taps32 t3[CH];
            float inG[CH], lf[CH], ga[CH], gb[CH];
            UpTaps o3[CH], t0[CH], t1[CH];
#pragma unroll
            for (int i = 0; i < CH; i++) {
                const int e = e0 + 256 * i;
                const uint32_t ec = (uint32_t)min(e, n2 - 1), ty = mul24(ec, m2) >> 22, tx = ec - mul24(ty, (uint32_t)n2x);
                ok[i] = e < n2, ti[i] = mul24(ty, U0H_T2) + tx;
                X2[i] = c2x0 + (int)tx, Y2[i] = c2y0 + (int)ty;
                ob[i] = (row2 + mul24(ty, (uint32_t)p.ws2) + (uint32_t)(X2[i] - p.lox2)) << 2;
                inG[i] = ld_su<float>(p.g2, (uint32_t)gm.K * ps2b + ob[i]);
                t3[i] = tap_bytes(row3, c3y0, ph.lox3, ph.ws3, X2[i], Y2[i]);
                o3[i] = taps_at(ph.out3, 0u, t3[i]);
            }
            __builtin_amdgcn_sched_barrier(0);
#pragma unroll
            for (int i = 0; i < CH; i++) {
                const float level = inG[i] * gm.Km1;
                const int li = dev::clampi((int)level, 0, gm.K - 2);
                lf[i] = level - (float)li;
                ga[i] = ld_su<float>(p.g2, (uint32_t)li * ps2b + ob[i]), gb[i] = ld_su<float>(p.g2, (uint32_t)(li + 1) * ps2b + ob[i]);
                t0[i] = taps_at(ph.g3, (uint32_t)li * ps3b, t3[i]);
                t1[i] = taps_at(ph.g3, (uint32_t)(li + 1) * ps3b, t3[i]);
            }
            __builtin_amdgcn_sched_barrier(0);
#pragma unroll
            for (int i = 0; i < CH; i++) {
                const float l0 = ga[i] - up_from(t0[i], X2[i], Y2[i]), l1 = gb[i] - up_from(t1[i], X2[i], Y2[i]);
                const float outL = dev::mad2(1.0f - lf[i], l0, lf[i], l1);
                if (ok[i]) s_out2[ti[i]] = up_from(o3[i], X2[i], Y2[i]) + outL;
            }
        }
        __syncthreads();
    }
    {
        const int n1 = U0_TW * th;
        constexpr uint32_t M1 = (4194304u + U0_TW - 1) / U0_TW;
        const uint32_t row1 = (uint32_t)((cy0 - p.loy1) * p.ws1), row2 = (uint32_t)((c2y0 - p.loy2) * p.ws2);
        for (int e0 = threadIdx.x; e0 < n1; e0 += 256 * CH) {
            int cx[CH], cy[CH];
            uint32_t ti[CH];
            bool ok[CH];
            Taps32 t2[CH];
            float inG[CH], lf[CH], ga[CH], gb[CH];
            UpTaps o2[CH], t0[CH], t1[CH];
#pragma unroll
            for (int i = 0; i < CH; i++) {
                const int e = e0 + 256 * i;
                const uint32_t ec = (uint32_t)min(e, n1 - 1), ty = mul24(ec, M1) >> 22, tx = ec - mul24(ty, U0_TW);
                ok[i] = e < n1 && cx0 + (int)tx <= p.rx1_1, ti[i] = mul24(ty, U0_TS) + tx;
                cx[i] = min(cx0 + (int)tx, p.rx1_1), cy[i] = cy0 + (int)ty;
                const uint32_t ob = (row1 + mul24(ty, (uint32_t)p.ws1) + (uint32_t)(cx[i] - p.lox1)) << 2;
                inG[i] = ld_su<float>(p.g1, (uint32_t)gm.K * ps1b + ob), ga[i] = ld_su<float>(p.g1, ob), gb[i] = ld_su<float>(p.g1, ps1b + ob);
                t2[i] = tap_bytes(row2, c2y0, p.lox2, p.ws2, cx[i], cy[i]);
                if (!ph.fuse2) o2[i] = taps_at(p.out2, 0u, t2[i]);
            }
            __builtin_amdgcn_sched_barrier(0);
#pragma unroll
            for (int i = 0; i < CH; i++) {
                const float level = inG[i] * gm.Km1;
                const int li = dev::clampi((int)level, 0, gm.K - 2);
                lf[i] = level - (float)li;
                t0[i] = taps_at(p.g2, (uint32_t)li * ps2b, t2[i]);
                t1[i] = taps_at(p.g2, (uint32_t)(li + 1) * ps2b, t2[i]);
            }
            __builtin_amdgcn_sched_barrier(0);
#pragma unroll
            for (int i = 0; i < CH; i++) {
                const float l0 = ga[i] - up_from(t0[i], cx[i], cy[i]), l1 = gb[i] - up_from(t1[i], cx[i], cy[i]);
                const float outL = dev::mad2(1.0f - lf[i], l0, lf[i], l1);
                float up2;
                if (ph.fuse2) {
                    const float *q = s_out2 + mul24((uint32_t)(dev::fdiv2(cy[i] - 1) - c2y0), U0H_T2) + (uint32_t)(dev::fdiv2(cx[i] - 1) - c2x0);
                    UpTaps t;
                    t.bb = q[0], t.ba = q[1], t.ab = q[U0H_T2], t.aa = q[U0H_T2 + 1];
                    up2 = up_from(t, cx[i], cy[i]);
                } else {
                    up2 = up_from(o2[i], cx[i], cy[i]);
                }
                if (ok[i]) s_out1[ti[i]] = up2 + outL;
            }
        }
    }
    __syncthreads();
    const int wave = __builtin_amdgcn_readfirstlane(threadIdx.x >> 6), lane = threadIdx.x & 63;
    const int x = bx * 256 + (wave & 1) * 128 + 2 * lane;
    const int y0 = by * (2 * p.RU) + (wave >> 1) * p.RU;
    if (y0 >= p.oh || x >= p.ow) return;
    const int y1 = min(y0 + p.RU, p.oh);
    const int X = p.ox0 + x;
    uint32_t inb = (uint32_t)(X - gm.ix0) * 2u, outb = (uint32_t)x * 2u, l0b = (uint32_t)(X - gm.ix0) * 4u;
    auto hl0 = [](float rm, float r0) {
        return dev::CANON_FMA ? __builtin_fmaf(r0, 0.75f, rm * 0.25f) : __builtin_fmaf(rm, 0.25f, r0 * 0.75f);
    };
    auto hl1 = [](float r0, float rp) { return __builtin_fmaf(rp, 0.25f, r0 * 0.75f); };
    auto vl = [](float uq, float ut, float wq, float wt) {
        return dev::CANON_FMA ? __builtin_fmaf(uq, wq, ut * wt) : __builtin_fmaf(uq, 0.25f, ut * 0.75f);
    };
    struct Frame {
        ushort2 c0, c1, c2;
        float2 l0;
    };
    auto fresh = [](uint32_t &v) {
        asm volatile("" : "+v"(v));
        return v;
    };
    auto load_frame = [&](int y, Frame &f) {
        const int yc = min(y, y1 - 1);
        const uint16_t *irow = p.in + (long)(p.oy0 + yc - gm.iy0) * p.in_sy;
        const uint32_t ib = fresh(inb);
        f.c0 = ld_frame2<NT>(irow + p.gco[0], ib), f.c1 = ld_frame2<NT>(irow + p.gco[1], ib), f.c2 = ld_frame2<NT>(irow + p.gco[2], ib);
        {
            const f2 *const lp = reinterpret_cast<const f2 *>(reinterpret_cast<const char *>(ph.outl0 + (size_t)yc * ph.l0_ws) + fresh(l0b));
            const f2 v = NT ? __builtin_nontemporal_load(lp) : *lp;
            f.l0 = make_float2(v.x, v.y);
        }
    };
    auto finish = [&](int y, const Frame &f) {
        const int Y = p.oy0 + min(y, y1 - 1);
        const int ya = dev::fdiv2(Y + 1), yb = dev::fdiv2(Y - 1);
        const bool yodd = dev::fmod2(Y) != 0;
        const int yq = (dev::CANON_FMA || yodd) ? ya : yb, yt = (dev::CANON_FMA || yodd) ? yb : ya;
        const float wq = yodd ? 0.25f : 0.75f, wt = yodd ? 0.75f : 0.25f;
        const float *oa = s_out1 + (yq - cy0) * U0_TS + (wave & 1) * 64 + lane;
        const float *ob = s_out1 + (yt - cy0) * U0_TS + (wave & 1) * 64 + lane;
        const float ax = oa[0], ay = oa[1], az = oa[2], bx = ob[0], by = ob[1], bz = ob[2];
        const float uo[2] = {vl(hl0(ax, ay), hl0(bx, by), wq, wt), vl(hl1(ay, az), hl1(by, bz), wq, wt)};
        const float outL[2] = {f.l0.x, f.l0.y};
        const uint16_t ch[3][2] = {{f.c0.x, f.c0.y}, {f.c1.x, f.c1.y}, {f.c2.x, f.c2.y}};
        uint16_t res[3][2];
#pragma unroll
        for (int i = 0; i < 2; i++) {
            const float gray = gray_from(ch[0][i], ch[1][i], ch[2][i]);
            const float og = (uo[i] + outL[i]) + 0.01f;
            const float gr = gray + 0.01f;
            const float n[3] = {(float)ch[0][i] * og, (float)ch[1][i] * og, (float)ch[2][i] * og};
            float q[3];
            div3_by(n, gr, q);
#pragma unroll
            for (int c = 0; c < 3; c++) res[c][i] = (uint16_t)__builtin_amdgcn_fmed3f(q[c], 0.0f, 65535.0f);
        }
        if (y < y1) {
            uint16_t *orow = p.out + (long)y * p.out_sy;
#pragma unroll
            for (int c = 0; c < 3; c++) st_frame2<NT>(reinterpret_cast<char *>(orow + (long)c * p.out_sc) + fresh(outb), res[c][0], res[c][1]);
        }
    };
    Frame f[U0H_PF];
#pragma unroll
    for (int i = 0; i < U0H_PF; i++) load_frame(y0 + i, f[i]);
    for (int y = y0; y < y1; y += U0H_PF) {
#pragma unroll
        for (int i = 0; i < U0H_PF; i++) {
            const Frame cur = f[i];
            load_frame(y + U0H_PF + i, f[i]);
            finish(y + i, cur);
        }
    }
}

const ArgTable ll_table("local_laplacian", {
    in_buf("input", T_U16, 3, {0, 1536, 0, 2560, 0, 3}),
    scalar_i32("levels").estimate(8),
    scalar_f32("alpha").estimate(1),
    scalar_f32("beta").estimate(1),
    out_buf("output", T_U16, 3, {0, 1536, 0, 2560, 0, 3}),
});

struct LlSwitches {
    std::optional<int> fuse_from, upchain_from, ru, units0, no_vec, emit, nt, fuse_up2, d01_exch, d01_pad_lds, no_lut_cache;
};
LlSwitches ll_switches() {
    const auto get = env_int;
    LlSwitches s;
    s.fuse_from = get("HLMI_LL_FUSE_FROM"), s.upchain_from = get("HLMI_LL_UPCHAIN_FROM");
    s.ru = get("HLMI_LL_RU"), s.units0 = get("HLMI_LL_UNITS0"), s.no_vec = get("HLMI_LL_NO_VEC");
    s.emit = get("HLMI_LL_EMIT"), s.nt = get("HLMI_LL_NT"), s.fuse_up2 = get("HLMI_LL_FUSE_UP2");
    s.d01_exch = get("HLMI_LL_D01_EXCH"), s.d01_pad_lds = get("HLMI_LL_D01_PAD_LDS"), s.no_lut_cache = get("HLMI_LL_NO_LUT_CACHE");
    return s;
}

int dev_clamp_ru(int ru) { return ru < 1 ? 1 : (ru > 300 ? 300 : ru); }

struct PairGeom {
    int S2;
    int Pbase;
    int nsx;
};
struct LlPlan {
    Geometry gm;
    Level lv[J];
    size_t off_g[J], off_out[J], off_l0, ws_floats;
    Up0Args u0;
    int nlut;
    int S, SU;
    int up_low;
    bool lut_cache;
    bool lut_lds;
    bool vec_frame;
    bool vec_in;
    bool b1;
    bool fast, fuse1, fuse2, emit, nt;
    bool d01;
    bool strip2;
    struct { PairGeom pg; bool exch; int nsy, nunits; size_t lds; } d0;
    struct { PairGeom pg; int nsy, nunits; } s2;
    int units_strip;
    size_t up0_lds;
};

struct LlBuffers {
    float *lut, *outl0;
    float *g[J], *outg[J];
};

PairGeom pair_geom(const Level &d, const Level &e) {
    PairGeom g;
    g.S2 = (d.odd || e.odd) ? 62 : 61;
    const int lim = e.odd ? 2 * e.lox - 1 : 2 * e.lox - 2;
    g.Pbase = min(d.lox, lim);
    const int hi1 = d.lox + d.w - 1, hi2 = e.lox + e.w - 1;
    const int x2_first = e.odd ? (g.Pbase + 1) / 2 + 0 : g.Pbase / 2 + 1;
    g.nsx = max((hi2 - x2_first + g.S2) / g.S2, (hi1 - g.Pbase + 2 * g.S2) / (2 * g.S2));
    return g;
}

void ll_plan(LlPlan &pl, const halide_buffer_t *input, const halide_buffer_t *output, int levels, float beta, const LlSwitches &sw,
             int stream_cus, int device_cus) {
    Up0Args &p = pl.u0;
    const int ow = p.ow = output->dim[0].extent, oh = p.oh = output->dim[1].extent, nc = p.nc = output->dim[2].extent;
    Geometry &gm = pl.gm;
    gm.K = levels;
    gm.half = (levels - 1) * 256;
    gm.Km1 = (float)(levels - 1);
    gm.inv_Km1 = 1.0f / gm.Km1;
    gm.ix0 = input->dim[0].min, gm.ix1 = gm.ix0 + input->dim[0].extent - 1;
    gm.iy0 = input->dim[1].min, gm.iy1 = gm.iy0 + input->dim[1].extent - 1;
    const int ic0 = input->dim[2].min, ic1 = ic0 + input->dim[2].extent - 1, iw = gm.ix1 - gm.ix0 + 1;

    Level *lv = pl.lv;
    int lox = gm.ix0, hix = gm.ix1, loy = gm.iy0, hiy = gm.iy1, so = gm.ix0;
    int rx0 = output->dim[0].min, rx1 = rx0 + ow - 1, ry0 = output->dim[1].min, ry1 = ry0 + oh - 1;
    size_t ws_floats = (size_t)(2 * gm.half + 1 + 63) & ~(size_t)63;
    for (int j = 0; j < J; j++) {
        Level &L = lv[j];
        L.lox = so, L.loy = loy, L.w = hix - so + 1, L.h = hiy - loy + 1;
        L.ws = (L.w + 3) & ~3;
        L.ps = ((size_t)L.ws * L.h + 3) & ~(size_t)3;
        L.rx0 = rx0, L.rx1 = rx1, L.ry0 = ry0, L.ry1 = ry1;
        if (j >= 1) {
            pl.off_g[j] = ws_floats;
            ws_floats += ((size_t)(levels + 1) * L.ps + 63) & ~(size_t)63;
            pl.off_out[j] = ws_floats;
            ws_floats += (L.ps + 63) & ~(size_t)63;
        }
        const bool odd = (so & 1) != 0;
        const int par = odd ? (floor_div(so + 1, 2) & 1) : ((floor_div(so, 2) + 1) & 1);
        lox = floor_div(lox - 2, 2), hix = floor_div(hix + 2, 2);
        loy = floor_div(loy - 2, 2), hiy = floor_div(hiy + 2, 2);
        so = lox - ((lox - par) & 1);
        if (j + 1 < J) {
            lv[j + 1].odd = odd;
            lv[j + 1].nsx = (hix - so + 1 + STRIP - 1) / STRIP;
        }
        rx0 = floor_div(rx0 - 1, 2), rx1 = floor_div(rx1 + 1, 2);
        ry0 = floor_div(ry0 - 1, 2), ry1 = floor_div(ry1 + 1, 2);
    }
    p.in = dev_ptr<uint16_t>(input), p.out = dev_ptr<uint16_t>(output);
    const uintptr_t din = (uintptr_t)p.in, dout = (uintptr_t)p.out;
    const long in_sy = p.in_sy = input->dim[1].stride, in_sc = input->dim[2].stride;
    const long out_sy = p.out_sy = output->dim[1].stride, out_sc = p.out_sc = output->dim[2].stride;
    p.ox0 = output->dim[0].min, p.oy0 = output->dim[1].min;
    p.beta = beta, pl.b1 = (beta == 1.0f);
    const int oc0 = output->dim[2].min;
    bool same = (nc == 3);
    for (int ch = 0; ch < 3; ch++) {
        p.gco[ch] = (long)((ch < ic0 ? ic0 : (ch > ic1 ? ic1 : ch)) - ic0) * in_sc;
        p.cco[ch] = ch < nc ? (long)(oc0 + ch - ic0) * in_sc : 0;
        if (p.cco[ch] != p.gco[ch]) same = false;
    }
    p.same_ch = same ? 1 : 0;
    pl.lut_cache = !sw.no_lut_cache.value_or(0);
    const bool lut_lds = pl.lut_lds = levels <= 15;
    const int nlut = pl.nlut = 2 * gm.half + 1;
    const size_t lut_sh = lut_lds ? sizeof(float) * nlut : 0;

    const int S = pl.S = [&] {
        const int v = sw.fuse_from.value_or(4);
        return (v >= J - 5 && v <= J - 2) ? v : J;
    }();
    const int SU = pl.SU = [&] {
        const int v = sw.upchain_from.value_or(S == 4 ? 3 : 0);
        return (v >= 1 && v <= J - 2) ? v : S;
    }();
    const bool partitioned = stream_cus < device_cus;
    bool vec_frame = (din % 4 == 0) && (dout % 4 == 0) && in_sy % 2 == 0 && out_sy % 2 == 0 && out_sc % 2 == 0 &&
                     ((p.ox0 - gm.ix0) % 2 == 0) && !sw.no_vec.value_or(0);
    for (int ch = 0; ch < 3; ch++) vec_frame = vec_frame && p.gco[ch] % 2 == 0 && p.cco[ch] % 2 == 0;
    pl.vec_frame = vec_frame;
    const bool vec_in = pl.vec_in = (din % 8 == 0) && in_sy % 4 == 0 && p.gco[0] % 4 == 0 && p.gco[1] % 4 == 0 && p.gco[2] % 4 == 0 &&
                                    iw % 4 == 0 && !sw.no_vec.value_or(0);
    const bool fast = pl.fast = vec_frame && same && nc == 3 && (ow & 1) == 0 && (p.ox0 & 1) == 0 &&
                                (double)(levels + 1) * (4.0 * (double)lv[1].ps) < 4.0e9;
    const bool fuse1 = pl.fuse1 = fast && SU >= 2;
    const bool d01 = pl.d01 = levels == KCH && lut_lds && vec_in;
    const bool emit = pl.emit = d01 && fast && fuse1 && lv[1].ws < (1 << 24) && sw.emit.value_or(1);
    const int RU = p.RU = dev_clamp_ru(sw.ru.value_or(emit ? (partitioned ? 32 : 8) : fuse1 ? (partitioned ? 32 : 16) : 8));
    pl.nt = sw.nt.value_or(partitioned ? 1 : 0) != 0;
    pl.fuse2 = emit && SU >= 3 && SU < J && sw.fuse_up2.value_or(1);
    pl.up_low = fuse1 ? (pl.fuse2 ? 3 : 2) : 1;
    pl.strip2 = d01 && S == 4;

    pl.off_l0 = ws_floats;
    if (emit) ws_floats += ((size_t)iw * (size_t)oh + 63) & ~(size_t)63;
    pl.ws_floats = ws_floats;

    constexpr int WPB = D0_THREADS / 64;
    if (!d01) {
        const Level &d = lv[1];
        const int target = sw.units0.value_or(8 * device_cus);
        pl.d0.nsy = max(1, min(max(target / d.nsx, (d.h + 63) / 64), max(1, d.h / 2)));
        pl.d0.nunits = d.nsx * pl.d0.nsy;
        pl.d0.lds = (lut_lds ? sizeof(float) * ((nlut + 1) & ~1) : 0) + sizeof(float2) * D0_THREADS * (KCH + 1);
    } else {
        const Level &e = lv[2];
        const PairGeom pg = pl.d0.pg = pair_geom(lv[1], e);
        const int target2 = sw.units0.value_or(emit && partitioned ? 10 * stream_cus : 8 * device_cus);
        bool exch = sw.d01_exch.value_or(1) != 0;
        int nwy = 0;
        auto ceil_div = [](int x, int y) { return (x + y - 1) / y; };
        if (exch) {
            const int nwy_max = max(1, target2 / (WPB * pg.nsx));
            const int n = max(2, (ceil_div(e.h, nwy_max) + 1 + 3) / 4);
            nwy = ceil_div(e.h, 4 * n - 1);
            exch = e.h / nwy >= 4;
        }
        pl.d0.exch = exch;
        if (exch) {
            pl.d0.nsy = nwy;
            pl.d0.nunits = pg.nsx * nwy * WPB;
        } else {
            pl.d0.nsy = max(1, min(max(target2 / pg.nsx, (e.h + 31) / 32), e.h));
            pl.d0.nunits = pg.nsx * pl.d0.nsy;
        }
        size_t sh2 = sizeof(float) * ((nlut + 1) & ~1) + sizeof(float2) * D01_STATE * (WPB + (exch ? WPB - 1 : 0));
        const int pad = sw.d01_pad_lds.value_or(emit && partitioned ? -1 : 0);
        constexpr size_t kHalfCuLds = 160 * 1024 / 2;
        if (pad < 0) sh2 = max(sh2, kHalfCuLds + 2048);
        else sh2 += (size_t)pad;
        pl.d0.lds = sh2;
    }
    if (pl.strip2) {
        pl.s2.pg = pair_geom(lv[3], lv[4]);
        pl.s2.nsy = (lv[4].h + S2_RPU - 1) / S2_RPU;
        pl.s2.nunits = (levels + 1) * pl.s2.pg.nsx * pl.s2.nsy;
    }
    pl.units_strip = 16 * device_cus;
    pl.up0_lds = emit   ? sizeof(float) * ((size_t)U0_TS * (RU + 2) + (size_t)U0H_T2 * (RU / 2 + 4))
                 : fast ? lut_sh + (fuse1 ? ((lut_lds && (nlut & 1)) ? 4 : 0) + sizeof(float) * U0_TS * (RU + 2) : 0)
                        : lut_sh;
}

struct LlLastCall {
    LlPlan pl;
    LlBuffers b;
    hipStream_t stream;
    bool out1_pending;
    bool out2_pending;
};
thread_local LlLastCall t_dbg = {};

StripArgs strip_args(const LlPlan &pl, const LlBuffers &b, int j) {
    const Level &sl = pl.lv[j], &d = pl.lv[j + 1];
    const int cols = d.nsx * (pl.gm.K + 1);
    StripArgs a;
    a.src = b.g[j], a.slox = sl.lox, a.sloy = sl.loy, a.sw = sl.w, a.sh = sl.h, a.sws = sl.ws, a.sps = sl.ps;
    a.dst = b.g[j + 1], a.Xs = d.lox, a.dloy = d.loy, a.dw = d.w, a.dh = d.h, a.dws = d.ws, a.dps = d.ps;
    a.nsx = d.nsx;
    a.nsy = max(1, min(max(pl.units_strip / cols, (d.h + 31) / 32), max(1, d.h / 2)));
    a.nunits = cols * a.nsy;
    return a;
}
CoarseArgs coarse_args(const LlPlan &pl, const LlBuffers &b, int from) {
    CoarseArgs ca;
    for (int dl = 0; from + dl < J; dl++) {
        const Level &L = pl.lv[from + dl];
        DevLevel &D = ca.lv[dl];
        D.g = b.g[from + dl], D.out = b.outg[from + dl], D.lox = L.lox, D.loy = L.loy, D.w = L.w, D.h = L.h, D.ws = L.ws, D.ps = (unsigned)L.ps;
        D.rx0 = L.rx0, D.ry0 = L.ry0, D.rw = L.rx1 - L.rx0 + 1, D.rh = L.ry1 - L.ry0 + 1;
    }
    ca.K = pl.gm.K, ca.Km1 = pl.gm.Km1;
    return ca;
}
UpArgs up_args(const LlPlan &pl, const LlBuffers &b, int j) {
    const Level &a = pl.lv[j], &c = pl.lv[j + 1];
    UpArgs u;
    u.g = b.g[j], u.ws = a.ws, u.ps = a.ps, u.lox = a.lox, u.loy = a.loy, u.gc = b.g[j + 1], u.outc = b.outg[j + 1], u.cws = c.ws, u.cps = c.ps;
    u.clox = c.lox, u.cloy = c.loy, u.rx0 = a.rx0, u.ry0 = a.ry0, u.rw = a.rx1 - a.rx0 + 1, u.rh = a.ry1 - a.ry0 + 1;
    u.K = pl.gm.K, u.Km1 = pl.gm.Km1, u.out = b.outg[j];
    return u;
}

struct LutKey {
    int device, levels;
    uint32_t alpha_bits;
};
static_assert(sizeof(LutKey) <= DERIVED_KEY_BYTES, "key does not fit an entry");
DerivedCache g_luts(8);


int ll_stage_table(void *uc, const DeviceCtx &ctx, const LlPlan &pl, float alpha, LlBuffers &b, DerivedUse &use) {
    const int nlut = pl.nlut;
    LutKey key;
    memset(&key, 0, sizeof key);
    key.device = ctx.device, key.levels = pl.gm.K;
    memcpy(&key.alpha_bits, &alpha, 4);
    int r = derived_acquire(uc, ctx, g_luts, &key, sizeof key, sizeof(float) * ((size_t)nlut + 64), pl.lut_cache, &use);
    if (r) return r;
    if (use.ptr) b.lut = (float *)use.ptr;
    if (use.fill) {
        HLMI_LAUNCH(uc, "ll_remap_lut", ctx.stream, ll_remap_lut, dim3((nlut + 255) / 256), dim3(256), 0, b.lut, pl.gm.half, alpha);
        use.filled(ctx.stream);
    }
    return 0;
}

int ll_stage_down0(void *uc, const LlPlan &pl, const LlBuffers &b, hipStream_t st) {
    const Geometry &gm = pl.gm;
    const Up0Args &f = pl.u0;
    const Level &d = pl.lv[1], &e = pl.lv[2];
    const int levels = gm.K, iw = gm.ix1 - gm.ix0 + 1;
    Levels lev;
    for (int k = 0; k < MAX_K; k++) lev.v[k] = (float)k * gm.inv_Km1;
    constexpr int WPB = D0_THREADS / 64;
    dim3 block(D0_THREADS);
    const double d0_bytes = 6.0 * iw * (gm.iy1 - gm.iy0 + 1) + 4.0 * (levels + 1) * d.w * d.h;
    if (!pl.d01) {
        dim3 grid((pl.d0.nunits + WPB - 1) / WPB);
        timing_note_bytes(d0_bytes);
        return with_flags([&](auto O, auto V, auto L, auto B) -> int {
            HLMI_LAUNCH(uc, "ll_down0", st, (ll_down0<O.value, V.value, L.value, B.value>), grid, block, pl.d0.lds, f.in, f.in_sy,
                        f.gco[0], f.gco[1], f.gco[2], gm, lev, f.beta, b.lut, b.g[1], d.lox, d.loy, d.w, d.h, d.ws, d.ps, d.nsx,
                        pl.d0.nsy, pl.d0.nunits);
            return 0;
        }, d.odd, pl.vec_in, pl.lut_lds, pl.b1);
    }
    D01Args a;
    a.in = f.in, a.in_sy = f.in_sy, a.co0 = f.gco[0], a.co1 = f.gco[1], a.co2 = f.gco[2], a.beta = f.beta, a.lut_g = b.lut;
    a.g1 = b.g[1], a.so1 = d.lox, a.loy1 = d.loy, a.w1 = d.w, a.h1 = d.h, a.ws1 = d.ws, a.ps1 = d.ps;
    a.g2 = b.g[2], a.so2 = e.lox, a.loy2 = e.loy, a.w2 = e.w, a.h2 = e.h, a.ws2 = e.ws, a.ps2 = e.ps;
    a.S2 = pl.d0.pg.S2, a.Pbase = pl.d0.pg.Pbase, a.nsx = pl.d0.pg.nsx, a.nsy = pl.d0.nsy, a.nunits = pl.d0.nunits;
    a.nsy_magic = a.nsy == 1 ? 0u : (unsigned)((1ull << 32) / (unsigned)a.nsy + 1ull);
    a.rows_base = e.h / a.nsy, a.rows_rem = e.h % a.nsy;
    dim3 grid((a.nunits + WPB - 1) / WPB);
    if (pl.emit) {
        timing_note_bytes(6.0 * iw * (gm.iy1 - gm.iy0 + 1) + 4.0 * iw * f.oh + 4.0 * 3.0 * d.w * d.h + 4.0 * (levels + 1) * e.w * e.h);
        D01EArgs ae;
        ae.d = a, ae.outl0 = b.outl0, ae.oy0 = f.oy0, ae.oh = f.oh;
        ae.nsx_magic = a.nsx == 1 ? 0u : (unsigned)((1ull << 32) / (unsigned)a.nsx + 1ull);
        return with_flags([&](auto O0, auto O1, auto B, auto EX, auto NT) -> int {
            HLMI_LAUNCH(uc, "ll_down01", st, (ll_down01e<O0.value, O1.value, B.value, EX.value, NT.value>), grid, block, pl.d0.lds, ae, gm, lev);
            return 0;
        }, d.odd, e.odd, pl.b1, pl.d0.exch, pl.nt);
    }
    timing_note_bytes(d0_bytes + 4.0 * (levels + 1) * e.w * e.h);
    return with_flags([&](auto O0, auto O1, auto B, auto EX) -> int {
        HLMI_LAUNCH(uc, "ll_down01", st, (ll_down01f<O0.value, O1.value, B.value, EX.value>), grid, block, pl.d0.lds, a, gm, lev);
        return 0;
    }, d.odd, e.odd, pl.b1, pl.d0.exch);
}

int ll_stage_down_rest(void *uc, const LlPlan &pl, const LlBuffers &b, hipStream_t st) {
    const Level *lv = pl.lv;
    const int levels = pl.gm.K, S = pl.S;
    if (pl.strip2) {
        const Level &sl = lv[2], &d = lv[3], &e = lv[4];
        Strip2Args a;
        a.src = b.g[2], a.slox = sl.lox, a.sloy = sl.loy, a.sw = sl.w, a.sh = sl.h, a.sws = sl.ws, a.sps = sl.ps;
        a.g1 = b.g[3], a.so1 = d.lox, a.loy1 = d.loy, a.w1 = d.w, a.h1 = d.h, a.ws1 = d.ws, a.ps1 = d.ps;
        a.g2 = b.g[4], a.so2 = e.lox, a.loy2 = e.loy, a.w2 = e.w, a.h2 = e.h, a.ws2 = e.ws, a.ps2 = e.ps;
        a.S2 = pl.s2.pg.S2, a.Pbase = pl.s2.pg.Pbase, a.nsx = pl.s2.pg.nsx, a.nsy = pl.s2.nsy, a.nunits = pl.s2.nunits;
        timing_note_bytes(4.0 * (levels + 1) * ((double)sl.w * sl.h + (double)d.w * d.h + (double)e.w * e.h));
        dim3 grid((a.nunits + 3) / 4), block(256);
        if (int r = with_flags([&](auto O0, auto O1) -> int {
                HLMI_LAUNCH(uc, "ll_down_strip2:2", st, (ll_down_strip2<O0.value, O1.value>), grid, block, 0, a);
                return 0;
            }, d.odd, e.odd)) return r;
    }
    for (int j = 1; j + 1 < J; j++) {
        if (pl.strip2 && (j == 2 || j == 3)) continue;
        if (j == S) {
            const CoarseArgs ca = coarse_args(pl, b, S);
            long total = 0;
            for (int dl = 1; S + dl < J; dl++) total += (long)(levels + 1) * lv[S + dl].w * lv[S + dl].h;
            const int ntx = (lv[J - 1].w + DM_T - 1) / DM_T, nty = (lv[J - 1].h + DM_T - 1) / DM_T;
            dim3 grid((unsigned)(ntx * nty * (levels + 1))), block(256);
            char nm[32];
            snprintf(nm, sizeof nm, "ll_down_multi:%d", S);
            timing_note_bytes(4.0 * ((double)(levels + 1) * lv[S].w * lv[S].h + (double)total));
            if (J - 1 - S == 4) HLMI_LAUNCH(uc, nm, st, (ll_down_multi<4>), grid, block, 0, ca, ntx, nty);
            else if (J - 1 - S == 3) HLMI_LAUNCH(uc, nm, st, (ll_down_multi<3>), grid, block, 0, ca, ntx, nty);
            else if (J - 1 - S == 2) HLMI_LAUNCH(uc, nm, st, (ll_down_multi<2>), grid, block, 0, ca, ntx, nty);
            else HLMI_LAUNCH(uc, nm, st, (ll_down_multi<1>), grid, block, 0, ca, ntx, nty);
            break;
        }
        if (j == 1 && pl.d01) continue;
        const StripArgs sa = strip_args(pl, b, j);
        dim3 grid((sa.nunits + 3) / 4), block(256);
        char nm[32];
        snprintf(nm, sizeof nm, "ll_down_strip:%d", j);
        timing_note_bytes(4.0 * (levels + 1) * ((double)lv[j].w * lv[j].h + (double)lv[j + 1].w * lv[j + 1].h));
        if (int r = with_flags([&](auto O) -> int {
                HLMI_LAUNCH(uc, nm, st, (ll_down_strip<O.value>), grid, block, 0, sa);
                return 0;
            }, lv[j + 1].odd)) return r;
    }
    return 0;
}

int ll_stage_up_coarse(void *uc, const LlPlan &pl, const LlBuffers &b, hipStream_t st) {
    const Level *lv = pl.lv;
    const int levels = pl.gm.K, SU = pl.SU;
    if (SU < J) {
        const CoarseArgs cu = coarse_args(pl, b, SU);
        const int ntx = (cu.lv[0].rw + UM_T - 1) / UM_T, nty = (cu.lv[0].rh + UM_T - 1) / UM_T;
        dim3 grid((unsigned)(ntx * nty)), block(256);
        char nm[32];
        snprintf(nm, sizeof nm, "ll_up_multi:%d", SU);
        {
            const double px = (double)cu.lv[0].rw * cu.lv[0].rh;
            timing_note_bytes(4.0 * 4.0 * px * (SU + 1 < J ? 4.0 / 3.0 : 1.0));
        }
        switch (J - 1 - SU) {
#define LL_UM(T) case T: HLMI_LAUNCH(uc, nm, st, (ll_up_multi<T>), grid, block, 0, cu, ntx); break;
            LL_UM(1) LL_UM(2) LL_UM(3) LL_UM(4) LL_UM(5) LL_UM(6)
#undef LL_UM
        }
    } else {
        const Level &t = lv[J - 1];
        int rw = t.rx1 - t.rx0 + 1, rh = t.ry1 - t.ry0 + 1;
        HLMI_LAUNCH(uc, "ll_top", st, ll_top, dim3((rw + 63) / 64, rh), dim3(64), 0, b.g[J - 1], t.ws, t.ps, t.lox, t.loy, t.rx0,
                    t.ry0, rw, rh, levels, pl.gm.Km1, b.outg[J - 1]);
    }
    for (int j = min(SU, J - 1) - 1; j >= pl.up_low; j--) {
        const UpArgs ua = up_args(pl, b, j);
        char nm[32];
        snprintf(nm, sizeof nm, "ll_up:%d", j);
        timing_note_bytes(4.0 * (4.0 * ua.rw * ua.rh + 3.0 * (lv[j + 1].rx1 - lv[j + 1].rx0 + 1) * (lv[j + 1].ry1 - lv[j + 1].ry0 + 1)));
        HLMI_LAUNCH(uc, nm, st, ll_up<false>, dim3((ua.rw + 255) / 256, ua.rh), dim3(256), 0, ua);
    }
    return 0;
}

int ll_stage_up0(void *uc, const LlPlan &pl, const LlBuffers &b, hipStream_t st) {
    const Geometry &gm = pl.gm;
    const Level *lv = pl.lv;
    const Level &c = lv[1];
    Up0Args p = pl.u0;
    const int ow = p.ow, oh = p.oh, nc = p.nc;
    p.lut_g = b.lut, p.g1 = b.g[1], p.out1 = b.outg[1];
    p.lox1 = c.lox, p.loy1 = c.loy, p.ws1 = c.ws, p.ps1 = c.ps;
    p.g2 = b.g[2], p.out2 = b.outg[2], p.lox2 = lv[2].lox, p.loy2 = lv[2].loy, p.ws2 = lv[2].ws, p.ps2 = lv[2].ps;
    p.rx1_1 = c.rx1, p.rx0_1 = c.rx0, p.ry0_1 = c.ry0, p.ry1_1 = c.ry1;
    dim3 grid((ow + 255) / 256, (oh + 2 * p.RU - 1) / (2 * p.RU)), block(256);
    const double n1 = (double)(c.rx1 - c.rx0 + 1) * (c.ry1 - c.ry0 + 1), n2 = (double)(lv[2].rx1 - lv[2].rx0 + 1) * (lv[2].ry1 - lv[2].ry0 + 1);
    if (pl.emit) {
        timing_note_bytes(2.0 * (3 + nc) * ow * oh + 4.0 * ow * oh + 4.0 * 3.0 * n1 + 4.0 * 3.0 * n2);
        Up0HArgs ph;
        ph.u = p, ph.outl0 = b.outl0, ph.l0_ws = gm.ix1 - gm.ix0 + 1;
        ph.fuse2 = pl.fuse2 ? 1 : 0;
        ph.g3 = b.g[3], ph.out3 = b.outg[3], ph.lox3 = lv[3].lox, ph.loy3 = lv[3].loy, ph.ws3 = lv[3].ws, ph.ps3 = lv[3].ps;
        return with_flags([&](auto NT) -> int {
            HLMI_LAUNCH(uc, "ll_up0", st, ll_up0h<NT.value>, grid, block, pl.up0_lds, ph, gm);
            return 0;
        }, pl.nt);
    }
    timing_note_bytes(2.0 * (3 + nc) * ow * oh + 4.0 * 3.0 * n1 + (pl.fuse1 ? 4.0 * 3.0 * n2 : 0.0));
    if (pl.fast) {
        return with_flags([&](auto L, auto B, auto F) -> int {
            HLMI_LAUNCH(uc, "ll_up0", st, (ll_up0f<L.value, B.value, F.value>), grid, block, pl.up0_lds, p, gm);
            return 0;
        }, pl.lut_lds, pl.b1, pl.fuse1);
    }
    return with_flags([&](auto V, auto L) -> int {
        HLMI_LAUNCH(uc, "ll_up0", st, (ll_up0<V.value, L.value>), grid, block, pl.up0_lds, p, gm);
        return 0;
    }, pl.vec_frame, pl.lut_lds);
}

}

extern "C" int local_laplacian(halide_buffer_t *input, int32_t levels, float alpha, float beta, halide_buffer_t *output) {
    void *uc = nullptr;
    const LlSwitches sw = ll_switches();
    BufArg args[2];
    ll_table.bufs(args, {input, output});
    int r = check_not_null(uc, args, 2);
    if (r) return r;
    if ((r = check_type_and_dims(uc, args, 2))) return r;
    if (any_bounds_query(args, 2)) {
        int mins[3], ext[3];
        for (int d = 0; d < 3; d++) mins[d] = output->dim[d].min, ext[d] = output->dim[d].extent;
        answer_query(input, mins, ext);
        answer_query(output, mins, ext);
        return 0;
    }
    if ((r = check_shapes(uc, args, 2))) return r;
    for (int d = 0; d < 3; d++) {
        if ((r = check_covers(uc, args[0], d, output->dim[d].min, output->dim[d].extent))) return r;
    }
    if (levels < 2) {
        return report(uc, halide_error_code_param_too_small, "Parameter levels is %d but must be at least 2", levels);
    }
    if (levels > (1 << 20)) {
        return report(uc, halide_error_code_param_too_large, "Parameter levels is %d but must be at most %d", levels, 1 << 20);
    }
    const int nc = output->dim[2].extent;
    if (nc > 3) {
        return report(uc, halide_error_code_constraint_violated, "Output buffer output has %d channels, at most 3 supported", nc);
    }

    DeviceCtx ctx;
    if ((r = to_device(uc, &ctx, args, 2))) return r;
    if (output->dim[0].extent == 0 || output->dim[1].extent == 0 || nc == 0) {
        mark_output_written(output);
        return 0;
    }

    LlPlan pl;
    ll_plan(pl, input, output, levels, beta, sw, stream_cu_count(ctx.device, ctx.stream), stream_cu_count(ctx.device, nullptr));

    void *ws = nullptr;
    if ((r = get_workspace(uc, ctx, pl.ws_floats * sizeof(float), &ws))) return r;
    float *wsf = (float *)ws;
    LlBuffers b;
    b.lut = wsf, b.outl0 = wsf + pl.off_l0;
    b.g[0] = b.outg[0] = nullptr;
    for (int j = 1; j < J; j++) b.g[j] = wsf + pl.off_g[j], b.outg[j] = wsf + pl.off_out[j];
    t_dbg.pl = pl, t_dbg.b = b, t_dbg.stream = ctx.stream;
    t_dbg.out1_pending = pl.fuse1, t_dbg.out2_pending = pl.fuse2;

    hipStream_t st = ctx.stream;
    DerivedUse table;
    if ((r = ll_stage_table(uc, ctx, pl, alpha, b, table)) || (r = ll_stage_down0(uc, pl, b, st)) || (r = ll_stage_down_rest(uc, pl, b, st)) ||
        (r = ll_stage_up_coarse(uc, pl, b, st)) || (r = ll_stage_up0(uc, pl, b, st))) {
        return r;
    }
    table.done(st);
    mark_output_written(output);
    return 0;
}

HLMI_ENTRY_AUTO(local_laplacian, ll_table.md)

extern "C" int hlmi_debug_ll_probe(unsigned long long *out32) {
#if HLMI_LL_PROBE
    if (hipDeviceSynchronize() != hipSuccess) return -1;
    if (hipMemcpyFromSymbol(out32, HIP_SYMBOL(g_probe), sizeof(unsigned long long) * 32) != hipSuccess) return -1;
    unsigned long long zero[32] = {};
    if (hipMemcpyToSymbol(HIP_SYMBOL(g_probe), zero, sizeof zero) != hipSuccess) return -1;
    return 1;
#else
    (void)out32;
    return 0;
#endif
}

extern "C" int hlmi_debug_ll_residency(unsigned long long *out16) {
#if HLMI_LL_RESIDENCY
    if (hipDeviceSynchronize() != hipSuccess) return -1;
    if (hipMemcpyFromSymbol(out16, HIP_SYMBOL(g_res_hist), sizeof(unsigned long long) * 16) != hipSuccess) return -1;
    unsigned long long zero[16] = {};
    if (hipMemcpyToSymbol(HIP_SYMBOL(g_res_hist), zero, sizeof zero) != hipSuccess) return -1;
    return 1;
#else
    (void)out16;
    return 0;
#endif
}

extern "C" int hlmi_debug_dpp_probe(void) {
    int *flag = nullptr, h = 0;
    if (hipMalloc(&flag, sizeof(int)) != hipSuccess) return -1;
    if (hipMemset(flag, 0, sizeof(int)) != hipSuccess) return -1;
    hipLaunchKernelGGL(ll_dpp_probe, dim3(1), dim3(64), 0, 0, flag);
    if (hipMemcpy(&h, flag, sizeof(int), hipMemcpyDeviceToHost) != hipSuccess) return -1;
    (void)hipFree(flag);
    return h;
}

extern "C" int hlmi_debug_div3_check(const float *n, const float *d, int count) {
    float *dn = nullptr, *dd = nullptr;
    int *bad = nullptr, h = -1;
    if (hipMalloc(&dn, sizeof(float) * count) != hipSuccess || hipMalloc(&dd, sizeof(float) * count) != hipSuccess ||
        hipMalloc(&bad, sizeof(int)) != hipSuccess) {
        return -1;
    }
    if (hipMemcpy(dn, n, sizeof(float) * count, hipMemcpyHostToDevice) != hipSuccess ||
        hipMemcpy(dd, d, sizeof(float) * count, hipMemcpyHostToDevice) != hipSuccess ||
        hipMemset(bad, 0, sizeof(int)) != hipSuccess) {
        return -1;
    }
    hipLaunchKernelGGL(ll_div3_check, dim3((count + 255) / 256), dim3(256), 0, 0, dn, dd, count, bad);
    if (hipMemcpy(&h, bad, sizeof(int), hipMemcpyDeviceToHost) != hipSuccess) h = -1;
    (void)hipFree(dn), (void)hipFree(dd), (void)hipFree(bad);
    return h;
}

extern "C" int hlmi_debug_local_laplacian_outg(int level, float *dst, int cap_floats, int *rw_out, int *rh_out) {
    LlLastCall &c = t_dbg;
    if (level < 1 || level >= J || !c.b.outg[level]) return -1;
    const Level &L = c.pl.lv[level];
    int rw = L.rx1 - L.rx0 + 1, rh = L.ry1 - L.ry0 + 1;
    if (rw_out) *rw_out = rw;
    if (rh_out) *rh_out = rh;
    if (!dst) return 0;
    if ((long)rw * rh > cap_floats) return -1;
    auto collapse = [&c](int j, bool sel) {
        const UpArgs ua = up_args(c.pl, c.b, j);
        with_flags([&](auto SEL) -> int {
            hipLaunchKernelGGL(ll_up<SEL.value>, dim3((ua.rw + 255) / 256, ua.rh), dim3(256), 0, c.stream, ua);
            return 0;
        }, sel);
        return hipGetLastError() == hipSuccess;
    };
    if ((level == 1 || level == 2) && c.out2_pending) {
        if (!collapse(2, false)) return -1;
        c.out2_pending = false;
    }
    if (level == 1 && c.out1_pending) {
        if (!collapse(1, c.pl.emit)) return -1;
        c.out1_pending = false;
    }
    if (hipStreamSynchronize(c.stream) != hipSuccess) return -1;
    const float *src = c.b.outg[level] + (size_t)(L.ry0 - L.loy) * L.ws + (L.rx0 - L.lox);
    if (hipMemcpy2D(dst, sizeof(float) * rw, src, sizeof(float) * L.ws, sizeof(float) * rw, rh, hipMemcpyDeviceToHost) !=
        hipSuccess) {
        return -1;
    }
    return 0;
}
```

Before: 115,700 Mpx/s.

## Emit level-1 Laplacian inside down01 kernel using LDS ring of level-2 values

Adds an EM1 path in which the fused level-0/1/2 downsampling kernel computes the level-1 Laplacian directly. It keeps a per-wave LDS ring of freshly computed level-2 Gaussian values and exchanges boundary rows between waves. The kernel then writes one float per level-1 pixel instead of storing three level-1 planes, and up0h reads that single plane instead of re-gathering g2 taps and LUT planes. The cost is more LDS, one fewer wave per SIMD via launch bounds, narrower strips, extra barriers and possibly a smaller RU chosen so everything fits in LDS.

```diff
diff --git a/halide_amd/csrc/local_laplacian.hip b/halide_amd/csrc/local_laplacian.hip
--- a/halide_amd/csrc/local_laplacian.hip
+++ b/halide_amd/csrc/local_laplacian.hip
@@ -668,20 +668,45 @@
     else walk(std::false_type{});
 }
 
+struct UpTaps {
+    float aa, ab, ba, bb;
+};
+__device__ __forceinline__ UpTaps up_taps(const float *__restrict__ f, int lox, int loy, int ws, int X, int Y) {
+    const int xa = dev::fdiv2(X + 1) - lox, xb = dev::fdiv2(X - 1) - lox;
+    const int ya = dev::fdiv2(Y + 1) - loy, yb = dev::fdiv2(Y - 1) - loy;
+    UpTaps t;
+    t.aa = f[(size_t)ya * ws + xa], t.ab = f[(size_t)ya * ws + xb];
+    t.ba = f[(size_t)yb * ws + xa], t.bb = f[(size_t)yb * ws + xb];
+    return t;
+}
+__device__ __forceinline__ float up_from(const UpTaps &t, int X, int Y) {
+    const float wx = (float)(dev::fmod2(X) * 2 + 1) * 0.25f, wy = (float)(dev::fmod2(Y) * 2 + 1) * 0.25f;
+    const float ua = dev::lerpf(t.aa, t.ab, wx);
+    const float ub = dev::lerpf(t.ba, t.bb, wx);
+    return dev::lerpf(ua, ub, wy);
+}
+__device__ __forceinline__ float up_at(const float *__restrict__ f, int lox, int loy, int ws, int X, int Y) {
+    return up_from(up_taps(f, lox, loy, ws, X, Y), X, Y);
+}
+
 struct D01EArgs {
     D01Args d;
     float *outl0;
     int oy0, oh;
     unsigned nsx_magic;
+    int last2;
 };
+constexpr int D01_RING = KCH * 2 * 64;
+constexpr int D01_PUB2 = KCH * 64;
+constexpr size_t d01_em1_lds_bytes() { return sizeof(float) * ((D0_THREADS / 64) * D01_RING + (D0_THREADS / 64 - 1) * D01_PUB2); }
 typedef float f2 __attribute__((ext_vector_type(2)));
 __device__ __forceinline__ f2 f2s(float v) { return f2{v, v}; }
 __device__ __forceinline__ f2 fma2(f2 a, f2 b, f2 c) { return __builtin_elementwise_fma(a, b, c); }
 __device__ __forceinline__ f2 mad_2(f2 a, f2 b, f2 c) { return dev::CANON_FMA ? fma2(a, b, c) : a * b + c; }
 __device__ __forceinline__ f2 mad2_2(f2 a, f2 b, f2 c, f2 d) { return dev::CANON_FMA ? fma2(a, b, c * d) : a * b + c * d; }
 
-template<bool ODD0, bool ODD1, bool B1, bool EXCH, bool NT>
-__global__ __launch_bounds__(D0_THREADS, 2) void ll_down01e(D01EArgs pe, Geometry gm, Levels lev) {
+template<bool ODD0, bool ODD1, bool B1, bool EXCH, bool NT, bool EM1>
+__global__ __launch_bounds__(D0_THREADS, EM1 ? 1 : 2) void ll_down01e(D01EArgs pe, Geometry gm, Levels lev) {
     const D01Args &p = pe.d;
     LL_RESIDENCY(0);
     extern __shared__ float slut[];
@@ -702,6 +727,7 @@
         A = GA + wave * n, B = min(A + n - 1, GB);
         if (A > GB) {
             __syncthreads();
+            if (EM1) __syncthreads();
             return;
         }
         self_halo = !(wave < 3 && A + n <= GB);
@@ -722,7 +748,8 @@
 #pragma unroll
     for (int i = 0; i < 4; i++) xo[i] = qs.oq + qs.sel[i];
     const bool edge_wave = __any(!qs.plain);
-    const int T0 = 2 * A - 1, T1 = self_halo ? 2 * B + 2 : 2 * B;
+    const bool ext1 = EM1 && self_halo && B < pe.last2;
+    const int T0 = 2 * A - 1, T1 = self_halo ? (ext1 ? 2 * B + 4 : 2 * B + 2) : 2 * B;
     const int Ts0 = max(EXCH ? 2 * A - 1 : 2 * A, p.loy1), Ts1 = min(EXCH ? 2 * B : 2 * B + 1, p.loy1 + p.h1 - 1);
     const int off1 = P - p.so1;
     const bool st1_ok = lane < p.S2 && off1 >= 0 && off1 < p.w1;
@@ -734,6 +761,10 @@
     f2 *st2 = reinterpret_cast<f2 *>(slut + ((2 * gm.half + 2) & ~1)) + wave * D01_STATE + lane;
     f2 *pub_all = reinterpret_cast<f2 *>(slut + ((2 * gm.half + 2) & ~1)) + (D0_THREADS / 64) * D01_STATE + lane;
     f2 *pub_mine = pub_all + (wave - 1) * D01_STATE, *pub_next = pub_all + wave * D01_STATE;
+    float *const ring = slut + ((2 * gm.half + 2) & ~1) + 2 * D01_STATE * ((D0_THREADS / 64) + (EXCH ? D0_THREADS / 64 - 1 : 0)) +
+                        wave * D01_RING + lane;
+    float *const pub2_mine = ring + ((D0_THREADS / 64) - wave) * D01_RING + (wave - 1) * D01_PUB2, *const pub2_next = pub2_mine + D01_PUB2;
+    const bool e1_ok = (ODD1 ? (lane >= 1 && lane <= p.S2) : (lane >= 2 && lane <= p.S2 + 1)) && off1 >= 0 && off1 < p.w1;
     const int lbase = gm.half - 256 * (KCH - 1);
     float level[KCH];
 #pragma unroll
@@ -918,6 +949,42 @@
             else *dst = f4_t{r[0], r[1], r[2], r[3]};
         }
     };
+    struct L1Row {
+        float2 a, b;
+        f2 k;
+    };
+    auto sel_row = [&](const f2 *row, f2 sK) {
+        const int lx = dev::clampi((int)(sK.x * gm.Km1), 0, KCH - 2), ly = dev::clampi((int)(sK.y * gm.Km1), 0, KCH - 2);
+        const float *fx = reinterpret_cast<const float *>(row) + (lx << 8), *fy = reinterpret_cast<const float *>(row) + (ly << 8) + 1;
+        L1Row r;
+        r.a = make_float2(fx[0], fy[0]), r.b = make_float2(fx[256], fy[256]), r.k = sK;
+        return r;
+    };
+    auto em1_pair = [&](const L1Row &r, int U, auto yodd_tag) {
+        constexpr int YP = decltype(yodd_tag)::value ? 1 : 0;
+        const int ob = ((U - 1) & 1) * 64, oa = 64 - ob;
+        auto px = [&](float ga, float gb, float inG, int coff, int xpar) {
+            const float level = inG * gm.Km1;
+            const int li = dev::clampi((int)level, 0, KCH - 2);
+            const float lf = level - (float)li;
+            const float *q = ring + (li << 7) + coff;
+            UpTaps t0, t1;
+            t0.bb = q[ob], t0.ba = q[ob + 1], t0.ab = q[oa], t0.aa = q[oa + 1];
+            t1.bb = q[128 + ob], t1.ba = q[128 + ob + 1], t1.ab = q[128 + oa], t1.aa = q[128 + oa + 1];
+            const float l0 = ga - up_from(t0, xpar, YP), l1 = gb - up_from(t1, xpar, YP);
+            return dev::mad2(1.0f - lf, l0, lf, l1);
+        };
+        return make_float2(px(r.a.x, r.b.x, r.k.x, -1, ODD1 ? 1 : 0), px(r.a.y, r.b.y, r.k.y, ODD1 ? -1 : 0, ODD1 ? 0 : 1));
+    };
+    auto em1_store = [&](int U, float2 vo, float2 ve) {
+        if (e1_ok) {
+            const int y = 2 * U - 1 - p.loy1;
+            float *drow = p.g1 + (long)y * p.ws1 + off1;
+            if (y >= 0 && y < p.h1) *reinterpret_cast<float2 *>(drow) = vo;
+            if (y + 1 >= 0 && y + 1 < p.h1) *reinterpret_cast<float2 *>(drow + p.ws1) = ve;
+        }
+    };
+    L1Row dl_o0 = {}, dl_o1 = {}, dl_e = {};
 #if HLMI_LL_PROBE
     unsigned long long pr_planes = 0, pr_emit = 0, pr_prep = 0, pr_steps = 0;
     LL_PROBE_T(pe0);
@@ -951,8 +1018,11 @@
         f2 lv[2][4], dy[2][2];
         f2 res[KCH + 1];
         f2 sa, sb;
-        const bool out2 = PH == 1 && T >= 2 * A + 2;
+        const bool out2 = PH == 1 && T >= 2 * A + 2 && (!EM1 || T <= 2 * B + 2);
         float *d2 = p.g2 + (size_t)(((T - 2) >> 1) - p.loy2) * p.ws2 + off2;
+        const int U = (T - 2) >> 1;
+        float *const ringU = ring + (U & 1) * 64;
+        const bool pub2 = EM1 && EXCH && publish && T == 2 * A + 2;
         LL_PROBE_T(ps0);
         auto level2 = [&](int k) {
             const f2 c = res[k];
@@ -971,6 +1041,10 @@
                 }
                 if (out2 && st2_ok) d2[(size_t)k * p.ps2] = o;
                 st2[(2 * k + 1) * 64] = c;
+                if (EM1 && k < KCH) {
+                    ringU[(2 * k) * 64] = o;
+                    if (pub2) pub2_mine[k * 64] = o;
+                }
             }
         };
         auto state_issue = [&](int k) {
@@ -995,7 +1069,7 @@
         __builtin_amdgcn_wave_barrier();
         __builtin_amdgcn_sched_barrier(0);
         f2 *const rowT = st2 + (PH == 0 ? 0 : 64), *const rowP = st2 + (PH == 0 ? 64 : 0);
-        const bool st1_row = T >= Ts0 && T <= Ts1;
+        const bool st1_row = !EM1 && T >= Ts0 && T <= Ts1;
         const bool em_rows = T >= 2 * A && T <= 2 * B + 1;
         EmPix eg[4];
         if (em_rows) {
@@ -1044,6 +1118,17 @@
             em_wait(fg[2], after1), ee[2] = em_arith(n1, 2, fg[2], row_even);
             em_wait(fg[3], after0), ee[3] = em_arith(n1, 3, fg[3], row_even);
         }
+        float2 x1o = make_float2(0.0f, 0.0f), x1e = x1o;
+        const bool em1_rows = EM1 && PH == 1 && U >= A + 1;
+        if (EM1) {
+            const L1Row cur = sel_row(rowT, sK);
+            if (PH == 0) {
+                dl_o1 = cur;
+            } else {
+                if (em1_rows) x1o = em1_pair(dl_o0, U, row_odd), x1e = em1_pair(dl_e, U, row_even);
+                dl_o0 = dl_o1, dl_e = cur;
+            }
+        }
         asm volatile("" ::: "memory");
         __builtin_amdgcn_sched_barrier(0);
         LL_PROBE_T(ps2);
@@ -1056,6 +1141,7 @@
             *reinterpret_cast<float2 *>(drow + p.ps1) = s1;
             *reinterpret_cast<f2 *>(drow + (size_t)KCH * p.ps1) = sK;
         }
+        if (em1_rows) em1_store(U, x1o, x1e);
         if (em_rows) {
             emit_store(2 * T - 1, eo);
             emit_store(2 * T, ee);
@@ -1081,6 +1167,7 @@
         step(std::integral_constant<int, 0>{}, T, p0, p1, p2, p3, a, b, a2, b2, first && publish ? pub_mine : nullptr);
         step(std::integral_constant<int, 1>{}, T + 1, p2, p3, p0, p1, a2, b2, a, b, first && publish ? pub_mine + 64 : nullptr);
         if (first) __syncthreads();
+        if (EM1 && EXCH && T == T0 + 2) __syncthreads();
     }
 #if HLMI_LL_PROBE
     LL_PROBE_T(pe1);
@@ -1101,6 +1188,22 @@
                 o = down4_tail(py, r.x, r.y, nx);
             }
             if (st2_ok) d2[(size_t)k * p.ps2] = o;
+            if (EM1 && k < KCH) ring[(2 * k + (B & 1)) * 64] = o;
+        }
+        if (EM1) {
+            asm volatile("" ::: "memory");
+            __builtin_amdgcn_wave_barrier();
+            const float2 ao = em1_pair(dl_o0, B, row_odd), ae = em1_pair(dl_e, B, row_even);
+            asm volatile("" ::: "memory");
+            __builtin_amdgcn_wave_barrier();
+#pragma unroll
+            for (int k = 0; k < KCH; k++) ring[(2 * k + ((B + 1) & 1)) * 64] = pub2_next[k * 64];
+            asm volatile("" ::: "memory");
+            __builtin_amdgcn_wave_barrier();
+            const L1Row r0 = sel_row(pub_next, pub_next[(2 * KCH) * 64]), r1 = sel_row(pub_next + 64, pub_next[(2 * KCH + 1) * 64]);
+            const float2 bo = em1_pair(r0, B + 1, row_odd), be = em1_pair(r1, B + 1, row_even);
+            em1_store(B, ao, ae);
+            em1_store(B + 1, bo, be);
         }
         {
             float eo[4], ee[4];
@@ -1250,26 +1353,6 @@
     }
 }
 
-struct UpTaps {
-    float aa, ab, ba, bb;
-};
-__device__ __forceinline__ UpTaps up_taps(const float *__restrict__ f, int lox, int loy, int ws, int X, int Y) {
-    const int xa = dev::fdiv2(X + 1) - lox, xb = dev::fdiv2(X - 1) - lox;
-    const int ya = dev::fdiv2(Y + 1) - loy, yb = dev::fdiv2(Y - 1) - loy;
-    UpTaps t;
-    t.aa = f[(size_t)ya * ws + xa], t.ab = f[(size_t)ya * ws + xb];
-    t.ba = f[(size_t)yb * ws + xa], t.bb = f[(size_t)yb * ws + xb];
-    return t;
-}
-__device__ __forceinline__ float up_from(const UpTaps &t, int X, int Y) {
-    const float wx = (float)(dev::fmod2(X) * 2 + 1) * 0.25f, wy = (float)(dev::fmod2(Y) * 2 + 1) * 0.25f;
-    const float ua = dev::lerpf(t.aa, t.ab, wx);
-    const float ub = dev::lerpf(t.ba, t.bb, wx);
-    return dev::lerpf(ua, ub, wy);
-}
-__device__ __forceinline__ float up_at(const float *__restrict__ f, int lox, int loy, int ws, int X, int Y) {
-    return up_from(up_taps(f, lox, loy, ws, X, Y), X, Y);
-}
 
 __device__ __forceinline__ float top_value(const float *__restrict__ g, size_t ps, size_t o, int K, float Km1) {
     float level = g[(size_t)K * ps + o] * Km1;
@@ -1322,6 +1405,13 @@
 __global__ __launch_bounds__(256) void ll_up(UpArgs a) {
     up_pixel<SEL>(a, blockIdx.x * blockDim.x + threadIdx.x, blockIdx.y);
 }
+__global__ __launch_bounds__(256) void ll_up_outl(UpArgs a) {
+    const int x = blockIdx.x * blockDim.x + threadIdx.x, y = blockIdx.y;
+    if (x >= a.rw || y >= a.rh) return;
+    const int X = a.rx0 + x, Y = a.ry0 + y;
+    const size_t o = (size_t)(Y - a.loy) * a.ws + (X - a.lox);
+    a.out[o] = up_at(a.outc, a.clox, a.cloy, a.cws, X, Y) + a.g[o];
+}
 
 struct DevLevel {
     float *g, *out;
@@ -1831,7 +1921,7 @@
 };
 constexpr int U0H_PF = 4;
 constexpr int U0H_T2 = 68;
-template<bool NT, int CH = 2>
+template<bool NT, bool EM1, int CH = 2>
 __global__ __launch_bounds__(256) void ll_up0h(Up0HArgs ph, Geometry gm) {
     const Up0Args &p = ph.u;
     LL_RESIDENCY(1);
@@ -1915,48 +2005,72 @@
         const int n1 = U0_TW * th;
         constexpr uint32_t M1 = (4194304u + U0_TW - 1) / U0_TW;
         const uint32_t row1 = (uint32_t)((cy0 - p.loy1) * p.ws1), row2 = (uint32_t)((c2y0 - p.loy2) * p.ws2);
-        for (int e0 = threadIdx.x; e0 < n1; e0 += 256 * CH) {
-            int cx[CH], cy[CH];
-            uint32_t ti[CH];
-            bool ok[CH];
-            Taps32 t2[CH];
-            float inG[CH], lf[CH], ga[CH], gb[CH];
-            UpTaps o2[CH], t0[CH], t1[CH];
-#pragma unroll
-            for (int i = 0; i < CH; i++) {
-                const int e = e0 + 256 * i;
-                const uint32_t ec = (uint32_t)min(e, n1 - 1), ty = mul24(ec, M1) >> 22, tx = ec - mul24(ty, U0_TW);
-                ok[i] = e < n1 && cx0 + (int)tx <= p.rx1_1, ti[i] = mul24(ty, U0_TS) + tx;
-                cx[i] = min(cx0 + (int)tx, p.rx1_1), cy[i] = cy0 + (int)ty;
-                const uint32_t ob = (row1 + mul24(ty, (uint32_t)p.ws1) + (uint32_t)(cx[i] - p.lox1)) << 2;
-                inG[i] = ld_su<float>(p.g1, (uint32_t)gm.K * ps1b + ob), ga[i] = ld_su<float>(p.g1, ob), gb[i] = ld_su<float>(p.g1, ps1b + ob);
-                t2[i] = tap_bytes(row2, c2y0, p.lox2, p.ws2, cx[i], cy[i]);
-                if (!ph.fuse2) o2[i] = taps_at(p.out2, 0u, t2[i]);
-            }
-            __builtin_amdgcn_sched_barrier(0);
-#pragma unroll
-            for (int i = 0; i < CH; i++) {
-                const float level = inG[i] * gm.Km1;
-                const int li = dev::clampi((int)level, 0, gm.K - 2);
-                lf[i] = level - (float)li;
-                t0[i] = taps_at(p.g2, (uint32_t)li * ps2b, t2[i]);
-                t1[i] = taps_at(p.g2, (uint32_t)(li + 1) * ps2b, t2[i]);
-            }
-            __builtin_amdgcn_sched_barrier(0);
-#pragma unroll
-            for (int i = 0; i < CH; i++) {
-                const float l0 = ga[i] - up_from(t0[i], cx[i], cy[i]), l1 = gb[i] - up_from(t1[i], cx[i], cy[i]);
-                const float outL = dev::mad2(1.0f - lf[i], l0, lf[i], l1);
-                float up2;
-                if (ph.fuse2) {
+        if constexpr (EM1) {
+            for (int e0 = threadIdx.x; e0 < n1; e0 += 256 * CH) {
+                int cx[CH], cy[CH];
+                uint32_t ti[CH];
+                bool ok[CH];
+                float outL[CH];
+#pragma unroll
+                for (int i = 0; i < CH; i++) {
+                    const int e = e0 + 256 * i;
+                    const uint32_t ec = (uint32_t)min(e, n1 - 1), ty = mul24(ec, M1) >> 22, tx = ec - mul24(ty, U0_TW);
+                    ok[i] = e < n1 && cx0 + (int)tx <= p.rx1_1, ti[i] = mul24(ty, U0_TS) + tx;
+                    cx[i] = min(cx0 + (int)tx, p.rx1_1), cy[i] = cy0 + (int)ty;
+                    outL[i] = ld_su<float>(p.g1, (row1 + mul24(ty, (uint32_t)p.ws1) + (uint32_t)(cx[i] - p.lox1)) << 2);
+                }
+#pragma unroll
+                for (int i = 0; i < CH; i++) {
                     const float *q = s_out2 + mul24((uint32_t)(dev::fdiv2(cy[i] - 1) - c2y0), U0H_T2) + (uint32_t)(dev::fdiv2(cx[i] - 1) - c2x0);
                     UpTaps t;
                     t.bb = q[0], t.ba = q[1], t.ab = q[U0H_T2], t.aa = q[U0H_T2 + 1];
-                    up2 = up_from(t, cx[i], cy[i]);
-                } else {
-                    up2 = up_from(o2[i], cx[i], cy[i]);
+                    if (ok[i]) s_out1[ti[i]] = up_from(t, cx[i], cy[i]) + outL[i];
                 }
-                if (ok[i]) s_out1[ti[i]] = up2 + outL;
+            }
+        } else {
+            for (int e0 = threadIdx.x; e0 < n1; e0 += 256 * CH) {
+                int cx[CH], cy[CH];
+                uint32_t ti[CH];
+                bool ok[CH];
+                Taps32 t2[CH];
+                float inG[CH], lf[CH], ga[CH], gb[CH];
+                UpTaps o2[CH], t0[CH], t1[CH];
+#pragma unroll
+                for (int i = 0; i < CH; i++) {
+                    const int e = e0 + 256 * i;
+                    const uint32_t ec = (uint32_t)min(e, n1 - 1), ty = mul24(ec, M1) >> 22, tx = ec - mul24(ty, U0_TW);
+                    ok[i] = e < n1 && cx0 + (int)tx <= p.rx1_1, ti[i] = mul24(ty, U0_TS) + tx;
+                    cx[i] = min(cx0 + (int)tx, p.rx1_1), cy[i] = cy0 + (int)ty;
+                    const uint32_t ob = (row1 + mul24(ty, (uint32_t)p.ws1) + (uint32_t)(cx[i] - p.lox1)) << 2;
+                    inG[i] = ld_su<float>(p.g1, (uint32_t)gm.K * ps1b + ob), ga[i] = ld_su<float>(p.g1, ob), gb[i] = ld_su<float>(p.g1, ps1b + ob);
+                    t2[i] = tap_bytes(row2, c2y0, p.lox2, p.ws2, cx[i], cy[i]);
+                    if (!ph.fuse2) o2[i] = taps_at(p.out2, 0u, t2[i]);
+                }
+                __builtin_amdgcn_sched_barrier(0);
+#pragma unroll
+                for (int i = 0; i < CH; i++) {
+                    const float level = inG[i] * gm.Km1;
+                    const int li = dev::clampi((int)level, 0, gm.K - 2);
+                    lf[i] = level - (float)li;
+                    t0[i] = taps_at(p.g2, (uint32_t)li * ps2b, t2[i]);
+                    t1[i] = taps_at(p.g2, (uint32_t)(li + 1) * ps2b, t2[i]);
+                }
+                __builtin_amdgcn_sched_barrier(0);
+#pragma unroll
+                for (int i = 0; i < CH; i++) {
+                    const float l0 = ga[i] - up_from(t0[i], cx[i], cy[i]), l1 = gb[i] - up_from(t1[i], cx[i], cy[i]);
+                    const float outL = dev::mad2(1.0f - lf[i], l0, lf[i], l1);
+                    float up2;
+                    if (ph.fuse2) {
+                        const float *q = s_out2 + mul24((uint32_t)(dev::fdiv2(cy[i] - 1) - c2y0), U0H_T2) + (uint32_t)(dev::fdiv2(cx[i] - 1) - c2x0);
+                        UpTaps t;
+                        t.bb = q[0], t.ba = q[1], t.ab = q[U0H_T2], t.aa = q[U0H_T2 + 1];
+                        up2 = up_from(t, cx[i], cy[i]);
+                    } else {
+                        up2 = up_from(o2[i], cx[i], cy[i]);
+                    }
+                    if (ok[i]) s_out1[ti[i]] = up2 + outL;
+                }
             }
         }
     }
@@ -2046,7 +2160,7 @@
 });
 
 struct LlSwitches {
-    std::optional<int> fuse_from, upchain_from, ru, units0, no_vec, emit, nt, fuse_up2, d01_exch, d01_pad_lds, no_lut_cache;
+    std::optional<int> fuse_from, upchain_from, ru, units0, no_vec, emit, nt, fuse_up2, d01_exch, d01_pad_lds, no_lut_cache, emit1;
 };
 LlSwitches ll_switches() {
     const auto get = env_int;
@@ -2055,6 +2169,7 @@
     s.ru = get("HLMI_LL_RU"), s.units0 = get("HLMI_LL_UNITS0"), s.no_vec = get("HLMI_LL_NO_VEC");
     s.emit = get("HLMI_LL_EMIT"), s.nt = get("HLMI_LL_NT"), s.fuse_up2 = get("HLMI_LL_FUSE_UP2");
     s.d01_exch = get("HLMI_LL_D01_EXCH"), s.d01_pad_lds = get("HLMI_LL_D01_PAD_LDS"), s.no_lut_cache = get("HLMI_LL_NO_LUT_CACHE");
+    s.emit1 = get("HLMI_LL_EMIT1");
     return s;
 }
 
@@ -2079,6 +2194,7 @@
     bool vec_in;
     bool b1;
     bool fast, fuse1, fuse2, emit, nt;
+    bool emit1;
     bool d01;
     bool strip2;
     struct { PairGeom pg; bool exch; int nsy, nunits; size_t lds; } d0;
@@ -2092,9 +2208,9 @@
     float *g[J], *outg[J];
 };
 
-PairGeom pair_geom(const Level &d, const Level &e) {
+PairGeom pair_geom(const Level &d, const Level &e, int fewer = 0) {
     PairGeom g;
-    g.S2 = (d.odd || e.odd) ? 62 : 61;
+    g.S2 = ((d.odd || e.odd) ? 62 : 61) - fewer;
     const int lim = e.odd ? 2 * e.lox - 1 : 2 * e.lox - 2;
     g.Pbase = min(d.lox, lim);
     const int hi1 = d.lox + d.w - 1, hi2 = e.lox + e.w - 1;
@@ -2183,17 +2299,38 @@
     const bool fuse1 = pl.fuse1 = fast && SU >= 2;
     const bool d01 = pl.d01 = levels == KCH && lut_lds && vec_in;
     const bool emit = pl.emit = d01 && fast && fuse1 && lv[1].ws < (1 << 24) && sw.emit.value_or(1);
-    const int RU = p.RU = dev_clamp_ru(sw.ru.value_or(emit ? (partitioned ? 32 : 8) : fuse1 ? (partitioned ? 32 : 16) : 8));
+    int RU = dev_clamp_ru(sw.ru.value_or(emit ? (partitioned ? 32 : 8) : fuse1 ? (partitioned ? 32 : 16) : 8));
     pl.nt = sw.nt.value_or(partitioned ? 1 : 0) != 0;
     pl.fuse2 = emit && SU >= 3 && SU < J && sw.fuse_up2.value_or(1);
     pl.up_low = fuse1 ? (pl.fuse2 ? 3 : 2) : 1;
+    constexpr bool kEmit1Default = true;
+    constexpr size_t kCuLds = 160 * 1024, kLdsGranule = 1280;
+    constexpr int WPB = D0_THREADS / 64;
+    auto lds_alloc = [](size_t bytes) { return (bytes + kLdsGranule - 1) / kLdsGranule * kLdsGranule; };
+    auto up0h_lds = [](int ru) { return sizeof(float) * ((size_t)U0_TS * (ru + 2) + (size_t)U0H_T2 * (ru / 2 + 4)); };
+    const size_t d01_lds_exch = sizeof(float) * ((nlut + 1) & ~1) + sizeof(float2) * D01_STATE * (2 * WPB - 1);
+    pl.emit1 = false;
+    {
+        const int e1 = sw.emit1.value_or(-1);
+        if (pl.fuse2 && (e1 > 0 || (e1 < 0 && partitioned && kEmit1Default))) {
+            const size_t d0 = lds_alloc(d01_lds_exch + d01_em1_lds_bytes());
+            auto fits = [&](int ru) { return d0 + 3 * lds_alloc(up0h_lds(ru)) <= kCuLds; };
+            int ru = RU;
+            if (partitioned && !sw.ru) {
+                ru &= ~3;
+                while (ru > 8 && !fits(ru)) ru -= 4;
+            }
+            pl.emit1 = e1 > 0 || fits(ru);
+            if (pl.emit1) RU = ru;
+        }
+    }
+    p.RU = RU;
     pl.strip2 = d01 && S == 4;
 
     pl.off_l0 = ws_floats;
     if (emit) ws_floats += ((size_t)iw * (size_t)oh + 63) & ~(size_t)63;
     pl.ws_floats = ws_floats;
 
-    constexpr int WPB = D0_THREADS / 64;
     if (!d01) {
         const Level &d = lv[1];
         const int target = sw.units0.value_or(8 * device_cus);
@@ -2202,7 +2339,7 @@
         pl.d0.lds = (lut_lds ? sizeof(float) * ((nlut + 1) & ~1) : 0) + sizeof(float2) * D0_THREADS * (KCH + 1);
     } else {
         const Level &e = lv[2];
-        const PairGeom pg = pl.d0.pg = pair_geom(lv[1], e);
+        const PairGeom pg = pl.d0.pg = pair_geom(lv[1], e, pl.emit1 ? (e.odd ? 1 : 2) : 0);
         const int target2 = sw.units0.value_or(emit && partitioned ? 10 * stream_cus : 8 * device_cus);
         bool exch = sw.d01_exch.value_or(1) != 0;
         int nwy = 0;
@@ -2222,6 +2359,7 @@
             pl.d0.nunits = pg.nsx * pl.d0.nsy;
         }
         size_t sh2 = sizeof(float) * ((nlut + 1) & ~1) + sizeof(float2) * D01_STATE * (WPB + (exch ? WPB - 1 : 0));
+        if (pl.emit1) sh2 += d01_em1_lds_bytes();
         const int pad = sw.d01_pad_lds.value_or(emit && partitioned ? -1 : 0);
         constexpr size_t kHalfCuLds = 160 * 1024 / 2;
         if (pad < 0) sh2 = max(sh2, kHalfCuLds + 2048);
@@ -2332,14 +2470,17 @@
     a.rows_base = e.h / a.nsy, a.rows_rem = e.h % a.nsy;
     dim3 grid((a.nunits + WPB - 1) / WPB);
     if (pl.emit) {
-        timing_note_bytes(6.0 * iw * (gm.iy1 - gm.iy0 + 1) + 4.0 * iw * f.oh + 4.0 * 3.0 * d.w * d.h + 4.0 * (levels + 1) * e.w * e.h);
+        timing_note_bytes(6.0 * iw * (gm.iy1 - gm.iy0 + 1) + 4.0 * iw * f.oh + 4.0 * (pl.emit1 ? 1.0 : 3.0) * d.w * d.h +
+                          4.0 * (levels + 1) * e.w * e.h);
         D01EArgs ae;
         ae.d = a, ae.outl0 = b.outl0, ae.oy0 = f.oy0, ae.oh = f.oh;
         ae.nsx_magic = a.nsx == 1 ? 0u : (unsigned)((1ull << 32) / (unsigned)a.nsx + 1ull);
-        return with_flags([&](auto O0, auto O1, auto B, auto EX, auto NT) -> int {
-            HLMI_LAUNCH(uc, "ll_down01", st, (ll_down01e<O0.value, O1.value, B.value, EX.value, NT.value>), grid, block, pl.d0.lds, ae, gm, lev);
+        ae.last2 = e.loy + e.h - 1;
+        return with_flags([&](auto O0, auto O1, auto B, auto EX, auto NT, auto E1) -> int {
+            HLMI_LAUNCH(uc, "ll_down01", st, (ll_down01e<O0.value, O1.value, B.value, EX.value, NT.value, E1.value>), grid, block, pl.d0.lds, ae,
+                        gm, lev);
             return 0;
-        }, d.odd, e.odd, pl.b1, pl.d0.exch, pl.nt);
+        }, d.odd, e.odd, pl.b1, pl.d0.exch, pl.nt, pl.emit1);
     }
     timing_note_bytes(d0_bytes + 4.0 * (levels + 1) * e.w * e.h);
     return with_flags([&](auto O0, auto O1, auto B, auto EX) -> int {
@@ -2443,15 +2584,15 @@
     dim3 grid((ow + 255) / 256, (oh + 2 * p.RU - 1) / (2 * p.RU)), block(256);
     const double n1 = (double)(c.rx1 - c.rx0 + 1) * (c.ry1 - c.ry0 + 1), n2 = (double)(lv[2].rx1 - lv[2].rx0 + 1) * (lv[2].ry1 - lv[2].ry0 + 1);
     if (pl.emit) {
-        timing_note_bytes(2.0 * (3 + nc) * ow * oh + 4.0 * ow * oh + 4.0 * 3.0 * n1 + 4.0 * 3.0 * n2);
+        timing_note_bytes(2.0 * (3 + nc) * ow * oh + 4.0 * ow * oh + 4.0 * (pl.emit1 ? 1.0 : 3.0) * n1 + 4.0 * 3.0 * n2);
         Up0HArgs ph;
         ph.u = p, ph.outl0 = b.outl0, ph.l0_ws = gm.ix1 - gm.ix0 + 1;
         ph.fuse2 = pl.fuse2 ? 1 : 0;
         ph.g3 = b.g[3], ph.out3 = b.outg[3], ph.lox3 = lv[3].lox, ph.loy3 = lv[3].loy, ph.ws3 = lv[3].ws, ph.ps3 = lv[3].ps;
-        return with_flags([&](auto NT) -> int {
-            HLMI_LAUNCH(uc, "ll_up0", st, ll_up0h<NT.value>, grid, block, pl.up0_lds, ph, gm);
+        return with_flags([&](auto NT, auto E1) -> int {
+            HLMI_LAUNCH(uc, "ll_up0", st, (ll_up0h<NT.value, E1.value>), grid, block, pl.up0_lds, ph, gm);
             return 0;
-        }, pl.nt);
+        }, pl.nt, pl.emit1);
     }
     timing_note_bytes(2.0 * (3 + nc) * ow * oh + 4.0 * 3.0 * n1 + (pl.fuse1 ? 4.0 * 3.0 * n2 : 0.0));
     if (pl.fast) {
@@ -2607,7 +2748,13 @@
         c.out2_pending = false;
     }
     if (level == 1 && c.out1_pending) {
-        if (!collapse(1, c.pl.emit)) return -1;
+        if (c.pl.emit1) {
+            const UpArgs ua = up_args(c.pl, c.b, 1);
+            hipLaunchKernelGGL(ll_up_outl, dim3((ua.rw + 255) / 256, ua.rh), dim3(256), 0, c.stream, ua);
+            if (hipGetLastError() != hipSuccess) return -1;
+        } else if (!collapse(1, c.pl.emit)) {
+            return -1;
+        }
         c.out1_pending = false;
     }
     if (hipStreamSynchronize(c.stream) != hipSuccess) return -1;
```

New measurement: 120,000 Mpx/s, median of 6. +3.7%, better.
